# ka9q/ka9q-radio

Measured on NVIDIA H100. Metric: input Msamples/s through forward+filter+inverse at N channels, higher is better.
Workload: dtype f32

## Files before the change

include/ka9q_gpu.h:

```cpp
#ifndef KA9Q_GPU_H
#define KA9Q_GPU_H 1
#include <stddef.h>
#include <stdint.h>

#ifdef __cplusplus
extern "C" {
#endif

enum kgpu_type { KGPU_COMPLEX = 1, KGPU_REAL = 2 };
enum kgpu_format {
  KGPU_FMT_F32 = 0,
  KGPU_FMT_I16 = 1
};
enum kgpu_chan_flags {
  KGPU_CHAN_ISB = 1,
  KGPU_CHAN_BEAM = 4
};

typedef struct kgpu_master kgpu_master;
typedef struct kgpu_bank kgpu_bank;

struct kgpu_ingest_stats {
  unsigned long long energy;
  unsigned int clips;
  unsigned int pad;
};

const char *kgpu_last_error(void);
unsigned long long kgpu_launch_count(void);
int kgpu_profile_enable(int on);
int kgpu_profile_reset(void);
int kgpu_profile_kernels(void);
const char *kgpu_profile_name(int kernel);
int kgpu_profile_get(int kernel, double *total_ms, long *count);
int kgpu_device_count(void);
int kgpu_set_device(int device);

kgpu_master *kgpu_master_create(int L, int M, int in_type);
kgpu_master *kgpu_master_create_ex(int L, int M, int in_type);
kgpu_master *kgpu_master_create_any(int L, int M, int in_type);
int kgpu_master_plan(int L, int M, int in_type, char *buf, int buflen);
void kgpu_master_destroy(kgpu_master *m);
int kgpu_master_points(kgpu_master const *m);
int kgpu_master_bins(kgpu_master const *m);
long kgpu_master_spec_stride(kgpu_master const *m);
int kgpu_master_describe(kgpu_master const *m, char *buf, int buflen);

int kgpu_forward(kgpu_master *m, const void *d_in, int fmt, float scale, int derandomize, int nblocks,
                 void *d_spec, void *d_stats, void *stream);

int kgpu_unpack_airspy12(const void *d_packed, long sampcount, void *d_i16, void *d_stats, void *stream);

enum kgpu_raw8 {
  KGPU_RAW_U8 = 1,
  KGPU_RAW_S8 = 2
};
struct kgpu_block_stats {
  unsigned long long energy;
  unsigned int overs;
  unsigned int over_samples;
};
struct kgpu_scale_change {
  long long at;
  double scale;
};
int kgpu_unpack8(const void *d_raw, int fmt, int in_type, long history, long L, int nblocks, double scale,
                 const struct kgpu_scale_change *d_chg, int nchg, long long a0, void *d_out, void *d_stats, void *stream);
int kgpu_scale_i16(const void *d_in, int in_type, long count, long long a0, double scale, const struct kgpu_scale_change *d_chg,
                   int nchg, int derandomize, float *d_out, void *stream);
int kgpu_block_stats_i16(const void *d_in, int in_type, long history, long L, int nblocks, int derandomize, int limit,
                         void *d_stats, void *stream);

enum kgpu_iq_fmt {
  KGPU_IQ_S8 = 1,
  KGPU_IQ_S16 = 2
};
struct kgpu_iq_write {
  long long first;
  long long n;
  double scale;
  long long m[5];
  long long overs;
  long long last_over;
};
struct kgpu_iq_state {
  double dc_i, dc_q, sinphi, imbalance, gain_i, gain_q, secphi, tanphi;
};
struct kgpu_iq_params {
  int kind;
  double dc_alpha;
  double gp;
};
struct kgpu_iq_record {
  long long seq;
  long long n, sum_i, sum_q;
  double i_energy, q_energy, dotprod;
  long long overs;
  long long since_over;
  struct kgpu_iq_state state;
};
int kgpu_iq_moments(const void *d_raw, int fmt, long long a0, long count, struct kgpu_iq_write *d_tab, int cap,
                    long long w_lo, int nw, void *stream);
int kgpu_iq_scan(const struct kgpu_iq_write *d_tab, struct kgpu_iq_state *d_coef, int cap, long long w_from, int nw,
                 const struct kgpu_iq_params *params, struct kgpu_iq_record *d_rec, void *stream);
int kgpu_iq_apply(const void *d_raw, int fmt, long long a0, long count, const struct kgpu_iq_write *d_tab,
                  const struct kgpu_iq_state *d_coef, int cap, long long w_lo, int nw, void *d_out, void *stream);

int kgpu_master_set_notches(kgpu_master *m, int const *bins, double const *alpha, int n);
int kgpu_apply_notches(kgpu_master *m, void *d_spec, int nblocks, void *stream);

kgpu_bank *kgpu_bank_create(kgpu_master *m, int capacity);
void kgpu_bank_destroy(kgpu_bank *b);
int kgpu_bank_define(kgpu_bank *b, int idx, int olen);
int kgpu_bank_define_ex(kgpu_bank *b, int idx, int olen, int out_type);
int kgpu_bank_define_wide(kgpu_bank *b, int idx, int olen, int out_type);
int kgpu_bank_define_huge(kgpu_bank *b, int idx, int olen, int out_type);
int kgpu_bank_define_ext(kgpu_bank *b, int idx, int olen, int out_type);
int kgpu_bank_define_any(kgpu_bank *b, int idx, int olen, int out_type);
int kgpu_chan_plan(int points, int out_type, char *buf, int buflen);
int kgpu_bank_set_filter(kgpu_bank *b, int idx, double low, double high, double kaiser_beta);
int kgpu_bank_set_filter_on(kgpu_bank *b, int idx, double low, double high, double kaiser_beta, void *stream);
int kgpu_bank_set_response(kgpu_bank *b, int idx, float const *response);
int kgpu_bank_get_response(kgpu_bank *b, int idx, float *response);
int kgpu_bank_set_shift(kgpu_bank *b, int idx, int shift);
int kgpu_bank_set_flags(kgpu_bank *b, int idx, int flags);
int kgpu_bank_enable(kgpu_bank *b, int idx, int enabled);
int kgpu_bank_set_weights(kgpu_bank *b, int idx, double alpha_re, double alpha_im, double beta_re, double beta_im);
int kgpu_bank_set_osc(kgpu_bank *b, int idx, int enable, double phase_cycles, double freq_cps, double rate_cps2,
                      double block_adj_cycles);
int kgpu_bank_get_osc_phase(kgpu_bank *b, int idx, double *phase_cycles);
int kgpu_bank_set_block_counter(kgpu_bank *b, long counter);
long kgpu_bank_block_counter(kgpu_bank const *b);
int kgpu_bank_channels(kgpu_bank const *b);
long kgpu_bank_out_stride(kgpu_bank const *b);
long kgpu_bank_out_offset(kgpu_bank const *b, int idx);
int kgpu_bank_run(kgpu_bank *b, const void *d_spec, int nblocks, void *d_out, void *stream);
int kgpu_bank_run_ex(kgpu_bank *b, const void *d_spec, int nblocks, void *d_out, long out_pitch, float *d_power, void *stream);
int kgpu_bank_run_one(kgpu_bank *b, int idx, const void *d_spec, void *d_out, void *stream);
int kgpu_bank_run_one_ex(kgpu_bank *b, int idx, const void *d_spec, void *d_out, float *d_power , void *stream);
int kgpu_bank_noise(kgpu_bank *b, const void *d_spec, int nblocks, double samprate, double *d_n0, void *stream);

int kgpu_bank_fm_front(kgpu_bank *b, const void *d_out, long out_pitch, int nblocks, float *d_baseband, double *d_stats, void *stream);

int kgpu_bank_commit(kgpu_bank *b, void *stream);
int kgpu_use_static_kernels(int on);
int kgpu_use_cols_tma(int on);
int kgpu_cols_tma_fits(int L, int M, int in_type, int fmt, const void *d_in);

int kgpu_plan_radices(int len, int *radices, int max);
int kgpu_plan_split(long n, int *n1, int *n2);
int kgpu_plan_radices_ex(int len, int *radices, int max);
int kgpu_plan_split_ex(long n, int *n1, int *n2);

int kgpu_multicast_copy(const void *d_src, void *mc_dst, unsigned long long bytes, int nctas, void *stream);

typedef struct kgpu_spectrum kgpu_spectrum;
kgpu_spectrum *kgpu_spectrum_create(int fft_n, int in_type, int bin_count);
int kgpu_spectrum_set_window(kgpu_spectrum *s, float const *window);
int kgpu_spectrum_run(kgpu_spectrum *s, const void *d_ring, long ring_samples, long end, int fmt, float scale,
                      const struct kgpu_scale_change *d_chg, int nchg, long long end_index, int derandomize, int shift, int fft_avg, double overlap, float *d_bins, void *stream);
int kgpu_spectrum_run_narrow(kgpu_spectrum *s, const void *d_ring, long ring_size, long ring_idx, int fft_avg,
                             double overlap, float *d_bins, int *fft_avg_used, void *stream);
int kgpu_spectrum_ring_append(void *d_ring, long ring_size, long ring_idx, const void *d_src, long olen, void *stream);
int kgpu_spectrum_describe(kgpu_spectrum const *s, char *buf, int buflen);
void kgpu_spectrum_destroy(kgpu_spectrum *s);
int kgpu_spectrum_plan(int fft_n, int in_type, char *buf, int buflen);

double kgpu_algorithmic_bytes(kgpu_master const *m, kgpu_bank const *b, int fmt);

#ifdef __cplusplus
}
#endif
#endif
```

ka9q_radio_b200/capi.py:

```python
from __future__ import annotations

import ctypes as C
import os
import subprocess
from pathlib import Path

PKG = Path(__file__).resolve().parent
LIB_PATH = PKG / "libka9qgpu.so"

KGPU_COMPLEX, KGPU_REAL = 1, 2
KGPU_FMT_F32, KGPU_FMT_I16 = 0, 1
KGPU_RAW_U8, KGPU_RAW_S8 = 1, 2
KGPU_CHAN_ISB = 1
KGPU_CHAN_BEAM = 4

_lib = None


class KgpuError(RuntimeError):
    pass


def build(force: bool = False) -> None:
    if force or not LIB_PATH.exists():
        subprocess.run(["make", "-C", str(PKG / "csrc"), "-s"], check=True)


def load() -> C.CDLL:
    global _lib
    if _lib is not None:
        return _lib
    if not LIB_PATH.exists():
        raise KgpuError(
            f"{LIB_PATH} is missing: build it with `make -C ka9q_radio_b200/csrc` "
            "(python -c 'import __graft_entry__ as g; g.build()'). There is no CPU fallback."
        )
    L = C.CDLL(str(LIB_PATH))
    vp, i, d, f, l = C.c_void_p, C.c_int, C.c_double, C.c_float, C.c_long
    L.kgpu_last_error.restype = C.c_char_p
    L.kgpu_launch_count.restype = C.c_ulonglong
    L.kgpu_set_device.argtypes = [i]
    L.kgpu_master_create.restype = vp
    L.kgpu_master_create.argtypes = [i, i, i]
    L.kgpu_master_create_ex.restype = vp
    L.kgpu_master_create_ex.argtypes = [i, i, i]
    L.kgpu_master_create_any.restype = vp
    L.kgpu_master_create_any.argtypes = [i, i, i]
    L.kgpu_master_plan.argtypes = [i, i, i, C.c_char_p, i]
    L.kgpu_master_destroy.argtypes = [vp]
    L.kgpu_master_points.argtypes = [vp]
    L.kgpu_master_bins.argtypes = [vp]
    L.kgpu_master_spec_stride.argtypes = [vp]
    L.kgpu_master_spec_stride.restype = l
    L.kgpu_master_describe.argtypes = [vp, C.c_char_p, i]
    L.kgpu_forward.argtypes = [vp, vp, i, f, i, i, vp, vp, vp]
    L.kgpu_master_set_notches.argtypes = [vp, vp, vp, i]
    L.kgpu_apply_notches.argtypes = [vp, vp, i, vp]
    L.kgpu_bank_create.restype = vp
    L.kgpu_bank_create.argtypes = [vp, i]
    L.kgpu_bank_destroy.argtypes = [vp]
    L.kgpu_bank_define.argtypes = [vp, i, i]
    L.kgpu_bank_set_filter.argtypes = [vp, i, d, d, d]
    L.kgpu_bank_set_filter_on.argtypes = [vp, i, d, d, d, vp]
    L.kgpu_bank_set_response.argtypes = [vp, i, vp]
    L.kgpu_bank_get_response.argtypes = [vp, i, vp]
    L.kgpu_bank_set_shift.argtypes = [vp, i, i]
    L.kgpu_bank_set_flags.argtypes = [vp, i, i]
    L.kgpu_bank_enable.argtypes = [vp, i, i]
    L.kgpu_bank_channels.argtypes = [vp]
    L.kgpu_bank_out_stride.argtypes = [vp]
    L.kgpu_bank_out_stride.restype = l
    L.kgpu_bank_out_offset.argtypes = [vp, i]
    L.kgpu_bank_out_offset.restype = l
    L.kgpu_bank_run.argtypes = [vp, vp, i, vp, vp]
    L.kgpu_bank_run_one.argtypes = [vp, i, vp, vp, vp]
    L.kgpu_bank_commit.argtypes = [vp, vp]
    L.kgpu_unpack_airspy12.argtypes = [vp, l, vp, vp, vp]
    L.kgpu_unpack8.argtypes = [vp, i, i, l, l, i, d, vp, i, C.c_longlong, vp, vp, vp]
    L.kgpu_block_stats_i16.argtypes = [vp, i, l, l, i, i, i, vp, vp]
    ll = C.c_longlong
    L.kgpu_iq_moments.argtypes = [vp, i, ll, l, vp, i, ll, i, vp]
    L.kgpu_iq_scan.argtypes = [vp, vp, i, ll, i, vp, vp, vp]
    L.kgpu_iq_apply.argtypes = [vp, i, ll, l, vp, vp, i, ll, i, vp, vp]
    L.kgpu_bank_define_ex.argtypes = [vp, i, i, i]
    L.kgpu_bank_define_wide.argtypes = [vp, i, i, i]
    L.kgpu_bank_define_huge.argtypes = [vp, i, i, i]
    L.kgpu_bank_define_ext.argtypes = [vp, i, i, i]
    L.kgpu_bank_define_any.argtypes = [vp, i, i, i]
    L.kgpu_chan_plan.argtypes = [i, i, C.c_char_p, i]
    L.kgpu_bank_set_weights.argtypes = [vp, i, d, d, d, d]
    L.kgpu_bank_set_osc.argtypes = [vp, i, i, d, d, d, d]
    L.kgpu_bank_get_osc_phase.argtypes = [vp, i, vp]
    L.kgpu_bank_set_block_counter.argtypes = [vp, l]
    L.kgpu_bank_block_counter.argtypes = [vp]
    L.kgpu_bank_block_counter.restype = l
    L.kgpu_bank_run_ex.argtypes = [vp, vp, i, vp, l, vp, vp]
    L.kgpu_bank_run_one_ex.argtypes = [vp, i, vp, vp, vp, vp]
    L.kgpu_bank_noise.argtypes = [vp, vp, i, d, vp, vp]
    L.kgpu_bank_fm_front.argtypes = [vp, vp, l, i, vp, vp, vp]
    L.kgpu_use_static_kernels.argtypes = [i]
    L.kgpu_use_cols_tma.argtypes = [i]
    L.kgpu_cols_tma_fits.argtypes = [i, i, i, i, vp]
    L.kgpu_profile_enable.argtypes = [i]
    L.kgpu_profile_name.argtypes = [i]
    L.kgpu_profile_name.restype = C.c_char_p
    L.kgpu_profile_get.argtypes = [i, vp, vp]
    L.kgpu_plan_radices.argtypes = [i, vp, i]
    L.kgpu_plan_split.argtypes = [l, vp, vp]
    L.kgpu_plan_radices_ex.argtypes = [i, vp, i]
    L.kgpu_plan_split_ex.argtypes = [l, vp, vp]
    L.kgpu_multicast_copy.argtypes = [vp, vp, C.c_ulonglong, i, vp]
    L.kgpu_algorithmic_bytes.argtypes = [vp, vp, i]
    L.kgpu_algorithmic_bytes.restype = d
    L.kgpu_spectrum_create.restype = vp
    L.kgpu_spectrum_create.argtypes = [i, i, i]
    L.kgpu_spectrum_set_window.argtypes = [vp, vp]
    L.kgpu_spectrum_run.argtypes = [vp, vp, l, l, i, f, vp, i, C.c_longlong, i, i, i, d, vp, vp]
    L.kgpu_spectrum_run_narrow.argtypes = [vp, vp, l, l, i, d, vp, vp, vp]
    L.kgpu_spectrum_ring_append.argtypes = [vp, l, l, vp, l, vp]
    L.kgpu_spectrum_describe.argtypes = [vp, C.c_char_p, i]
    L.kgpu_spectrum_destroy.argtypes = [vp]
    L.kgpu_spectrum_plan.argtypes = [i, i, C.c_char_p, i]
    _lib = L
    return L


def exported_symbols() -> list[str]:
    import re

    hdr = (PKG.parent / "include" / "ka9q_gpu.h").read_text()
    hdr = re.sub(r"/\*.*?\*/", " ", hdr, flags=re.S)
    return sorted(set(re.findall(r"\b(kgpu_[a-z0-9_]+)\s*\(", hdr)))


def profile_snapshot() -> dict[str, tuple[float, int]]:
    L = load()
    out = {}
    for k in range(L.kgpu_profile_kernels()):
        ms, cnt = C.c_double(0), C.c_long(0)
        L.kgpu_profile_get(k, C.cast(C.pointer(ms), C.c_void_p), C.cast(C.pointer(cnt), C.c_void_p))
        out[L.kgpu_profile_name(k).decode()] = (ms.value, cnt.value)
    return out


def plan_radices(length: int, extended: bool = False) -> list[int]:
    out = (C.c_int * 16)()
    fn = load().kgpu_plan_radices_ex if extended else load().kgpu_plan_radices
    n = fn(length, C.cast(out, C.c_void_p), 16)
    if n < 0:
        raise KgpuError(f"length {length} cannot be planned")
    return [out[k] for k in range(n)]


def plan_split(n: int, extended: bool = False) -> tuple[int, int]:
    a, b = C.c_int(0), C.c_int(0)
    fn = load().kgpu_plan_split_ex if extended else load().kgpu_plan_split
    if fn(n, C.cast(C.pointer(a), C.c_void_p), C.cast(C.pointer(b), C.c_void_p)) != 0:
        raise KgpuError(f"{n} points cannot be split")
    return a.value, b.value


def check(rc: int, what: str = "") -> int:
    if rc < 0:
        raise KgpuError(f"{what}: {load().kgpu_last_error().decode()}")
    return rc


def unpack8(d_raw: int, fmt: int, in_type: int, history: int, L: int, nblocks: int, scale: float, d_out: int,
            d_stats: int = 0, stream: int = 0) -> None:
    check(load().kgpu_unpack8(d_raw, fmt, in_type, history, L, nblocks, scale, None, 0, 0, d_out, d_stats or None,
                              stream or None), "kgpu_unpack8")


def block_stats_i16(d_in: int, in_type: int, history: int, L: int, nblocks: int, d_stats: int, derandomize: bool = False,
                    limit: int = 32767, stream: int = 0) -> None:
    check(load().kgpu_block_stats_i16(d_in, in_type, history, L, nblocks, int(derandomize), limit, d_stats, stream or None),
          "kgpu_block_stats_i16")


KGPU_IQ_S8, KGPU_IQ_S16 = 1, 2
IQ_HACKRF, IQ_FUNCUBE = 1, 2


class IqParams(C.Structure):
    _fields_ = [("kind", C.c_int), ("dc_alpha", C.c_double), ("gp", C.c_double)]


def iq_moments(d_raw: int, fmt: int, a0: int, count: int, d_tab: int, cap: int, w_lo: int, nw: int, stream: int = 0) -> None:
    check(load().kgpu_iq_moments(d_raw, fmt, a0, count, d_tab, cap, w_lo, nw, stream or None), "kgpu_iq_moments")


def iq_scan(d_tab: int, d_coef: int, cap: int, w_from: int, nw: int, kind: int, dc_alpha: float, gp: float, d_rec: int,
            stream: int = 0) -> None:
    p = IqParams(kind, dc_alpha, gp)
    check(load().kgpu_iq_scan(d_tab, d_coef, cap, w_from, nw, C.byref(p), d_rec, stream or None), "kgpu_iq_scan")


def iq_apply(d_raw: int, fmt: int, a0: int, count: int, d_tab: int, d_coef: int, cap: int, w_lo: int, nw: int, d_out: int,
             stream: int = 0) -> None:
    check(load().kgpu_iq_apply(d_raw, fmt, a0, count, d_tab, d_coef, cap, w_lo, nw, d_out, stream or None), "kgpu_iq_apply")


MASTER_DIRECT, MASTER_EXTENDED, MASTER_BLUESTEIN = 0, 1, 2


def plan_master(L: int, M: int, in_type: int) -> tuple[int, str]:
    buf = C.create_string_buffer(512)
    return check(load().kgpu_master_plan(L, M, in_type, buf, 512), "kgpu_master_plan"), buf.value.decode()


CHAN_DIRECT, CHAN_WIDE, CHAN_HUGE, CHAN_EXTENDED, CHAN_BLUESTEIN = 0, 1, 2, 3, 4


def chan_plan(points: int, out_type: int = KGPU_COMPLEX) -> tuple[int, str]:
    buf = C.create_string_buffer(512)
    return check(load().kgpu_chan_plan(points, out_type, buf, 512), "kgpu_chan_plan"), buf.value.decode()


class Master:

    def __init__(self, L: int, M: int, in_type: int, extended: bool = False, any_length: bool = False):
        self.lib = load()
        if any_length:
            what = "kgpu_master_create_any"
        else:
            what = "kgpu_master_create_ex" if extended else "kgpu_master_create"
        self.h = getattr(self.lib, what)(L, M, in_type)
        if not self.h:
            raise KgpuError(f"{what}: " + self.lib.kgpu_last_error().decode())
        self.L, self.M, self.in_type = L, M, in_type
        self.N = self.lib.kgpu_master_points(self.h)
        self.bins = self.lib.kgpu_master_bins(self.h)
        self.spec_stride = self.lib.kgpu_master_spec_stride(self.h)

    def describe(self) -> str:
        buf = C.create_string_buffer(512)
        self.lib.kgpu_master_describe(self.h, buf, 512)
        return buf.value.decode()

    def forward(self, d_in: int, fmt: int, scale: float, nblocks: int, d_spec: int, stream: int = 0,
                derandomize: bool = False, d_stats: int = 0) -> None:
        check(self.lib.kgpu_forward(self.h, d_in, fmt, scale, int(derandomize), nblocks, d_spec, d_stats or None,
                                    stream or None), "kgpu_forward")

    def set_notches(self, bins, alpha=0.01) -> None:
        bins = list(bins) + [0]
        n = len(bins)
        b = (C.c_int * n)(*bins)
        a = (C.c_double * n)(*([alpha] * n))
        check(self.lib.kgpu_master_set_notches(self.h, C.cast(b, C.c_void_p), C.cast(a, C.c_void_p), n), "set_notches")

    def apply_notches(self, d_spec: int, nblocks: int, stream: int = 0) -> None:
        check(self.lib.kgpu_apply_notches(self.h, d_spec, nblocks, stream or None), "kgpu_apply_notches")

    def close(self):
        if self.h:
            self.lib.kgpu_master_destroy(self.h)
            self.h = None


class Bank:

    def __init__(self, master: Master, capacity: int):
        self.lib = load()
        self.m = master
        self.h = self.lib.kgpu_bank_create(master.h, capacity)
        if not self.h:
            raise KgpuError("kgpu_bank_create: " + self.lib.kgpu_last_error().decode())

    def define(self, idx, olen, out_type=KGPU_COMPLEX) -> int:
        return check(self.lib.kgpu_bank_define_ex(self.h, idx, olen, out_type), "kgpu_bank_define_ex")

    def define_wide(self, idx, olen, out_type=KGPU_COMPLEX) -> int:
        return check(self.lib.kgpu_bank_define_wide(self.h, idx, olen, out_type), "kgpu_bank_define_wide")

    def define_huge(self, idx, olen, out_type=KGPU_COMPLEX) -> int:
        return check(self.lib.kgpu_bank_define_huge(self.h, idx, olen, out_type), "kgpu_bank_define_huge")

    def define_ext(self, idx, olen, out_type=KGPU_COMPLEX) -> int:
        return check(self.lib.kgpu_bank_define_ext(self.h, idx, olen, out_type), "kgpu_bank_define_ext")

    def define_any(self, idx, olen, out_type=KGPU_COMPLEX) -> int:
        return check(self.lib.kgpu_bank_define_any(self.h, idx, olen, out_type), "kgpu_bank_define_any")

    def set_weights(self, idx, i_weight=1.0, q_weight=0.0):
        a = 0.5 * complex(i_weight) - 1j * complex(q_weight)
        b = 0.5 * complex(i_weight) + 1j * complex(q_weight)
        check(self.lib.kgpu_bank_set_weights(self.h, idx, a.real, a.imag, b.real, b.imag), "kgpu_bank_set_weights")

    def set_osc(self, idx, enable, phase=0.0, freq=0.0, rate=0.0, block_adj=0.0):
        check(self.lib.kgpu_bank_set_osc(self.h, idx, int(enable), phase, freq, rate, block_adj), "kgpu_bank_set_osc")

    def osc_phase(self, idx) -> float:
        v = C.c_double(0)
        check(self.lib.kgpu_bank_get_osc_phase(self.h, idx, C.cast(C.pointer(v), C.c_void_p)), "kgpu_bank_get_osc_phase")
        return v.value

    @property
    def block_counter(self) -> int:
        return self.lib.kgpu_bank_block_counter(self.h)

    @block_counter.setter
    def block_counter(self, v: int):
        check(self.lib.kgpu_bank_set_block_counter(self.h, int(v)), "kgpu_bank_set_block_counter")

    def fm_front(self, d_out: int, nblocks: int, d_baseband: int, d_stats: int, stream: int = 0):
        check(self.lib.kgpu_bank_fm_front(self.h, d_out, 0, nblocks, d_baseband, d_stats, stream or None), "kgpu_bank_fm_front")

    def noise(self, d_spec: int, nblocks: int, samprate: float, d_n0: int, stream: int = 0):
        check(self.lib.kgpu_bank_noise(self.h, d_spec, nblocks, samprate, d_n0, stream or None), "kgpu_bank_noise")

    def set_filter(self, idx, low, high, beta):
        check(self.lib.kgpu_bank_set_filter(self.h, idx, low, high, beta), "kgpu_bank_set_filter")

    def set_response(self, idx, resp):
        import numpy as np

        r = np.ascontiguousarray(resp, np.complex64)
        check(self.lib.kgpu_bank_set_response(self.h, idx, r.ctypes.data), "kgpu_bank_set_response")

    def get_response(self, idx, points):
        import numpy as np

        r = np.empty(points, np.complex64)
        check(self.lib.kgpu_bank_get_response(self.h, idx, r.ctypes.data), "kgpu_bank_get_response")
        return r

    def set_shift(self, idx, shift):
        check(self.lib.kgpu_bank_set_shift(self.h, idx, int(shift)), "kgpu_bank_set_shift")

    def set_flags(self, idx, flags):
        check(self.lib.kgpu_bank_set_flags(self.h, idx, int(flags)), "kgpu_bank_set_flags")

    def enable(self, idx, on=True):
        check(self.lib.kgpu_bank_enable(self.h, idx, int(on)), "kgpu_bank_enable")

    @property
    def out_stride(self) -> int:
        return self.lib.kgpu_bank_out_stride(self.h)

    def out_offset(self, idx) -> int:
        return self.lib.kgpu_bank_out_offset(self.h, idx)

    def run(self, d_spec: int, nblocks: int, d_out: int, stream: int = 0, d_power: int = 0):
        check(self.lib.kgpu_bank_run_ex(self.h, d_spec, nblocks, d_out, 0, d_power or None, stream or None), "kgpu_bank_run")

    def run_one(self, idx, d_spec: int, d_out: int, stream: int = 0):
        check(self.lib.kgpu_bank_run_one(self.h, idx, d_spec, d_out, stream or None), "kgpu_bank_run_one")

    def algorithmic_bytes(self, fmt) -> float:
        return self.lib.kgpu_algorithmic_bytes(self.m.h, self.h, fmt)

    def close(self):
        if self.h:
            self.lib.kgpu_bank_destroy(self.h)
            self.h = None


SPECTRUM_R2C, SPECTRUM_COMPLEX, SPECTRUM_BLUESTEIN = 0, 1, 2


def spectrum_plan(fft_n: int, in_type: int) -> tuple[int, str]:
    buf = C.create_string_buffer(256)
    return check(load().kgpu_spectrum_plan(fft_n, in_type, buf, 256), "kgpu_spectrum_plan"), buf.value.decode()


def spectrum_ring_append(ring, ring_idx: int, block, stream: int = 0) -> int:
    import torch

    if not (ring.is_cuda and ring.is_contiguous() and ring.dtype == torch.float32 and ring.shape[-1] == 2):
        raise ValueError("ring must be a contiguous float32 CUDA tensor of (re, im) pairs")
    size = ring.numel() // 2
    if isinstance(block, int):
        src, n = None, block
    else:
        if not (block.is_cuda and block.is_contiguous() and block.dtype == torch.float32 and block.shape[-1] == 2):
            raise ValueError("block must be a contiguous float32 CUDA tensor of (re, im) pairs")
        src, n = block.data_ptr(), block.numel() // 2
    check(load().kgpu_spectrum_ring_append(ring.data_ptr(), size, int(ring_idx), src, n, stream or None),
          "kgpu_spectrum_ring_append")
    return (int(ring_idx) + n) % size


class Spectrum:

    def __init__(self, fft_n: int, in_type: int, bin_count: int):
        self.lib = load()
        self.h = self.lib.kgpu_spectrum_create(fft_n, in_type, bin_count)
        if not self.h:
            raise KgpuError("kgpu_spectrum_create: " + self.lib.kgpu_last_error().decode())
        self.fft_n, self.in_type, self.bin_count = fft_n, in_type, bin_count

    def describe(self) -> str:
        buf = C.create_string_buffer(256)
        self.lib.kgpu_spectrum_describe(self.h, buf, 256)
        return buf.value.decode()

    def set_window(self, window) -> None:
        import numpy as np

        w = np.ascontiguousarray(window, np.float32)
        if w.shape != (self.fft_n,):
            raise ValueError(f"window needs {self.fft_n} floats")
        check(self.lib.kgpu_spectrum_set_window(self.h, w.ctypes.data), "kgpu_spectrum_set_window")

# ... 37 lines not shown
```

ka9q_radio_b200/csrc/fft_static.cuh:

```cuda
#pragma once
#include "fft_radix.cuh"

namespace kfft {

template <int LEN, int... RS> struct SPlan {
  static constexpr int len = LEN;
  static constexpr int nst = sizeof...(RS);
  static constexpr int rad_arr[sizeof...(RS) > 0 ? sizeof...(RS) : 1] = {RS...};
  static constexpr int rad(int i) { return rad_arr[i]; }
  static constexpr int nsub(int i) {
    int n = LEN;
    for (int k = 0; k < i; k++) n /= rad_arr[k];
    return n;
  }
  static constexpr int stride(int i) { return nsub(i) / rad_arr[i]; }
  static constexpr int tw_off(int i) {
    int o = 0;
    for (int k = 0; k < i; k++)
      if (stride(k) > 1) o += (rad_arr[k] - 1) * stride(k);
    return o;
  }
  static constexpr bool valid() {
    int p = 1;
    for (int k = 0; k < nst; k++) p *= rad_arr[k];
    return p == LEN;
  }
};

template <class P, int I = 0> struct SlotOf {
  static __device__ __forceinline__ int run(int rem) {
    constexpr int R = P::rad(I), S = P::stride(I);
    int const q = rem / R;
    return (rem - q * R) * S + SlotOf<P, I + 1>::run(q);
  }
};
template <class P> struct SlotOf<P, P::nst> {
  static __device__ __forceinline__ int run(int) { return 0; }
};
template <class P> __device__ __forceinline__ int static_slot(int k) { return SlotOf<P>::run(k); }

template <class P> constexpr int static_tw_count() { return P::tw_off(P::nst); }

__device__ __forceinline__ int ldg_stream_b32(int const *p) {
  int v;
  asm volatile("ld.global.nc.L1::no_allocate.b32 %0, [%1];" : "=r"(v) : "l"(p));
  return v;
}
__device__ __forceinline__ float2 ldg_stream_f2(float2 const *p) {
  float2 v;
  asm volatile("ld.global.nc.L1::no_allocate.v2.f32 {%0, %1}, [%2];" : "=f"(v.x), "=f"(v.y) : "l"(p));
  return v;
}

template <class P, int I> struct StageGeom {
  static constexpr int R = P::rad(I), NSUB = P::nsub(I), S = P::stride(I), NB = P::len / R;
  static __device__ __forceinline__ void split(int u, int &b, int &j) {
    if (S == 1) {
      b = u;
      j = 0;
    } else {
      b = u / S;
      j = u - b * S;
    }
  }
};

template <class P, bool INV, int I, bool TWS, int ILP>
__device__ __forceinline__ void static_stage(float2 *__restrict__ col, float2 const *__restrict__ tw, int lane) {
  using G = StageGeom<P, I>;
  constexpr int R = G::R, NSUB = G::NSUB, S = G::S, NB = G::NB, NL = 32;
  constexpr int ITERS = (NB + NL - 1) / NL;
  float2 const *twi = tw + P::tw_off(I);
#pragma unroll
  for (int it0 = 0; it0 < ITERS; it0 += ILP) {
    float2 x[ILP][R];
    float2 *p[ILP];
    int jj[ILP];
    bool ok[ILP];
#pragma unroll
    for (int q = 0; q < ILP; q++) {
      int const u = lane + NL * (it0 + q);
      ok[q] = (it0 + q < ITERS) && ((NB % NL == 0) || it0 + q + 1 < ITERS || u < NB);
      int b, j;
      G::split(ok[q] ? u : 0, b, j);
      jj[q] = j;
      p[q] = col + b * NSUB + j;
      if (ok[q]) {
#pragma unroll
        for (int m = 0; m < R; m++) x[q][m] = p[q][m * S];
      }
    }
#pragma unroll
    for (int q = 0; q < ILP; q++) {
      if (ok[q]) {
        Dft<R, INV>::run(x[q]);
        if (S > 1) {
#pragma unroll
          for (int t = 1; t < R; t++) {
            float2 const w = TWS ? twi[(t - 1) * S + jj[q]] : __ldg(twi + (t - 1) * S + jj[q]);
            x[q][t] = INV ? cmulc(x[q][t], w) : cmul(x[q][t], w);
          }
        }
      }
    }
#pragma unroll
    for (int q = 0; q < ILP; q++) {
      if (ok[q]) {
#pragma unroll
        for (int t = 0; t < R; t++) p[q][t * S] = x[q][t];
      }
    }
  }
}

template <class P, bool INV, bool TWS = false, int ILP = 1, int I = 0> struct StaticFft {
  static __device__ __forceinline__ void run(float2 *col, float2 const *tw, int lane) {
    static_stage<P, INV, I, TWS, (P::rad(I) <= 12 ? ILP : 1)>(col, tw, lane);
    __syncwarp();
    StaticFft<P, INV, TWS, ILP, I + 1>::run(col, tw, lane);
  }
};
template <class P, bool INV, bool TWS, int ILP> struct StaticFft<P, INV, TWS, ILP, P::nst> {
  static __device__ __forceinline__ void run(float2 *, float2 const *, int) {}
};

__device__ __forceinline__ uint32_t smem_u32(void const *p) { return (uint32_t)__cvta_generic_to_shared(p); }
__device__ __forceinline__ void mbar_init(uint64_t *bar, int count) {
  asm volatile("mbarrier.init.shared::cta.b64 [%0], %1;" ::"r"(smem_u32(bar)), "r"(count));
}
__device__ __forceinline__ void mbar_fence_init() { asm volatile("fence.mbarrier_init.release.cluster;" ::: "memory"); }
__device__ __forceinline__ void mbar_expect_tx(uint64_t *bar, uint32_t bytes) {
  asm volatile("mbarrier.arrive.expect_tx.shared::cta.b64 _, [%0], %1;" ::"r"(smem_u32(bar)), "r"(bytes) : "memory");
}
__device__ __forceinline__ void bulk_g2s(void *dst, void const *src, uint32_t bytes, uint64_t *bar) {
  asm volatile("cp.async.bulk.shared::cluster.global.mbarrier::complete_tx::bytes [%0], [%1], %2, [%3];" ::"r"(smem_u32(dst)),
               "l"(src), "r"(bytes), "r"(smem_u32(bar))
               : "memory");
}
__device__ __forceinline__ void tensor_g2s_3d(void *dst, void const *map, int x, int y, int z, uint64_t *bar) {
  asm volatile("cp.async.bulk.tensor.3d.shared::cluster.global.tile.mbarrier::complete_tx::bytes [%0], [%1, {%2, %3, %4}], [%5];"
               ::"r"(smem_u32(dst)), "l"(map), "r"(x), "r"(y), "r"(z), "r"(smem_u32(bar))
               : "memory");
}
__device__ __forceinline__ void mbar_wait(uint64_t *bar, uint32_t parity) {
  asm volatile(
      "{\n\t.reg .pred p;\n\t"
      "WAIT_%=:\n\t"
      "mbarrier.try_wait.parity.shared::cta.b64 p, [%0], %1;\n\t"
      "@p bra DONE_%=;\n\t"
      "bra WAIT_%=;\n\t"
      "DONE_%=:\n\t}" ::"r"(smem_u32(bar)),
      "r"(parity)
      : "memory");
}

}
```

ka9q_radio_b200/csrc/fwd_cols_r36.cuh:

```cuda
#pragma once
#include <cuda.h>

#include "static_kernels_v2.cuh"

namespace kfft {

struct ColsR36Tables {
  float2 const *tw0;
  float2 const *twA;
  float2 const *twB;
};

__device__ __forceinline__ float2 r36_power(float2 const (&wb)[6], float2 const (&wa)[6], int t) {
  int const a = t / 6, b = t - 6 * a;
  if (a == 0) return wb[b];
  if (b == 0) return wa[a];
  return cmul(wa[a], wb[b]);
}

struct ColsR36Shape {
  static constexpr int BLK = 38, CP = 1378, T = 288;
  static constexpr size_t smem = sizeof(float2) * (size_t)(8 * CP + 360 + 80);
};

struct ColsR36Tma {
  static constexpr int BOX_ROWS = 216;
  static constexpr int F32_BOX_BYTES = BOX_ROWS * 64;
  static constexpr int I16_BOX_WORDS = 12, I16_BOX_BYTES = BOX_ROWS * I16_BOX_WORDS * 4;
  static constexpr int I16_ODD_OFF = 3 * I16_BOX_BYTES;
  static constexpr uint32_t bytes(int fmt) { return fmt == 0 ? 6 * F32_BOX_BYTES : 6 * I16_BOX_BYTES; }
};
static_assert(ColsR36Tma::bytes(0) + 112 <= sizeof(float2) * 8 * ColsR36Shape::CP &&
              ColsR36Tma::bytes(1) + 112 <= sizeof(float2) * 8 * ColsR36Shape::CP, "the raw tile lies in the float tile");
static_assert(ColsR36Tma::F32_BOX_BYTES % 128 == 0 && ColsR36Tma::I16_BOX_BYTES % 128 == 0, "box destinations 128-B aligned");

template <int FMT>
__device__ __forceinline__ float2 r36_ingest(int raw, int row, int col, int n2, Pass1Args const &a, unsigned long long &energy,
                                             unsigned int &clips) {
  int lo, hi;
  unpack_i16(raw, lo, hi);
  if (FMT == 2) {
    if (a.derandomize) {
      lo ^= (lo & 1) ? 0xfffffffe : 0;
      hi ^= (hi & 1) ? 0xfffffffe : 0;
    }
    if (a.stats && (long)row * n2 + col >= a.first_new) {
      energy += (unsigned long long)(lo * lo) + (unsigned long long)(hi * hi);
      clips += (lo > 32766 || lo < -32766) + (hi > 32766 || hi < -32766);
    }
  }
  return make_float2(i32_to_f32(lo), i32_to_f32(hi));
}

__device__ __forceinline__ void r36_stage0_store(float2 (&x)[36], float2 const *s_tw0, float2 *d, int ul) {
  constexpr int R = 36, BLK = ColsR36Shape::BLK;
  float2 wb[6], wa[6];
#pragma unroll
  for (int b = 1; b < 6; b++) {
    wb[b] = s_tw0[(b - 1) * 36 + ul];
    wa[b] = s_tw0[(4 + b) * 36 + ul];
  }
  d[0] = x[0];
#pragma unroll
  for (int t = 1; t < R; t++) d[t * BLK] = cmul(x[t], r36_power(wb, wa, t));
}

template <int FMT, int N2C, bool TMA>
__device__ __forceinline__ void fwd_cols_r36_body(Pass1Args const &a, ColsR36Tables const &tb, CUtensorMap const *tmap) {
  constexpr int R = 36, BLK = ColsR36Shape::BLK, CP = ColsR36Shape::CP;
  extern __shared__ __align__(16) unsigned char smem_raw[];
  float2 *tile = reinterpret_cast<float2 *>(smem_raw);
  float2 *s_tw0 = tile + 8 * CP;
  float2 *s_twB = s_tw0 + 360;
  __shared__ __align__(8) uint64_t tbar;
  int const tid = threadIdx.x;
  int const c = tid & 7, ul = tid >> 3;
  int const c0 = blockIdx.x * 8, blk = blockIdx.y;
  int const n2 = N2C ? N2C : a.n2;
  int const ld = N2C ? (N2C + 15) / 16 * 16 : a.mid_ld;
  int const ncols = min(8, n2 - c0);
  bool const col_ok = c < ncols;
  int const n2g = c0 + c;
  float2 *mycol = tile + c * CP;
  unsigned char *const rtile = smem_raw + ((0u - smem_u32(smem_raw)) & 127u);
  if (tid == 0) {
    mbar_init(&tbar, 1);
    mbar_fence_init();
    if constexpr (TMA) {
      using T = ColsR36Tma;
      mbar_expect_tx(&tbar, 360 * 8 + 80 * 8 + T::bytes(FMT));
      if (FMT == 0) {
#pragma unroll
        for (int k = 0; k < 6; k++) tensor_g2s_3d(rtile + k * T::F32_BOX_BYTES, tmap, 2 * c0, k * T::BOX_ROWS, blk, &tbar);
      } else {
#pragma unroll
        for (int k = 0; k < 3; k++) {
          tensor_g2s_3d(rtile + k * T::I16_BOX_BYTES, tmap, c0, k * T::BOX_ROWS, blk, &tbar);
          tensor_g2s_3d(rtile + T::I16_ODD_OFF + k * T::I16_BOX_BYTES, tmap, n2 + c0 - (n2 & 2), k * T::BOX_ROWS, blk, &tbar);
        }
      }
    } else {
      mbar_expect_tx(&tbar, 360 * 8 + 80 * 8);
    }
    bulk_g2s(s_tw0, tb.tw0, 360 * 8, &tbar);
    bulk_g2s(s_twB, tb.twB + (long)c0 * 10, 80 * 8, &tbar);
  }
  __syncthreads();
  float2 const twA = col_ok ? ldg_stream_f2(tb.twA + (long)n2g * 36 + ul) : make_float2(1.f, 0.f);

  unsigned long long energy = 0;
  unsigned int clips = 0;
  if constexpr (TMA) {
    float2 x[R];
    mbar_wait(&tbar, 0);
    if (col_ok) {
      if (FMT == 0) {
        float2 const *src = reinterpret_cast<float2 const *>(rtile) + ul * 8 + c;
#pragma unroll
        for (int m = 0; m < R; m++) x[m] = src[R * 8 * m];
      } else {
        using T = ColsR36Tma;
        int const odd = ul & 1;
        int const *src = reinterpret_cast<int const *>(rtile + odd * T::I16_ODD_OFF) + (ul >> 1) * T::I16_BOX_WORDS + c +
                         odd * (n2 & 2);
#pragma unroll
        for (int m = 0; m < R; m++)
          x[m] = r36_ingest<FMT>(src[(R / 2) * T::I16_BOX_WORDS * m], ul + R * m, n2g, n2, a, energy, clips);
      }
      Dft<R, false>::run(x);
    }
    __syncthreads();
    if (col_ok) r36_stage0_store(x, s_tw0, mycol + ul, ul);
  } else if (col_ok) {
    float2 x[R];
    if (FMT == 0) {
      float2 const *src = reinterpret_cast<float2 const *>(a.in) + (long)blk * a.hop + n2g + (long)ul * n2;
#pragma unroll
      for (int m = 0; m < R; m++) x[m] = ldg_stream_f2(src + (long)(R * m) * n2);
    } else {
      int const *src = reinterpret_cast<int const *>(a.in) + (long)blk * a.hop + n2g + (long)ul * n2;
      int raw[R];
#pragma unroll
      for (int m = 0; m < R; m++) raw[m] = ldg_stream_b32(src + (long)(R * m) * n2);
#pragma unroll
      for (int m = 0; m < R; m++) x[m] = r36_ingest<FMT>(raw[m], ul + R * m, n2g, n2, a, energy, clips);
    }
    mbar_wait(&tbar, 0);
    Dft<R, false>::run(x);
    r36_stage0_store(x, s_tw0, mycol + ul, ul);
  } else {
    mbar_wait(&tbar, 0);
  }
  if (FMT == 2 && a.stats) {
#pragma unroll
    for (int o = 16; o > 0; o >>= 1) {
      energy += __shfl_xor_sync(0xffffffffu, energy, o);
      clips += __shfl_xor_sync(0xffffffffu, clips, o);
    }
    if ((tid & 31) == 0 && (energy | clips)) {
      atomicAdd(&a.stats[blk].energy, energy);
      atomicAdd(&a.stats[blk].clips, clips);
    }
  }
  __syncthreads();

  if (col_ok) {
    float2 x[R];
    float4 const *p4 = reinterpret_cast<float4 const *>(mycol + ul * BLK);
#pragma unroll
    for (int m = 0; m < R / 2; m++) {
      float4 const v = p4[m];
      x[2 * m] = make_float2(v.x, v.y);
      x[2 * m + 1] = make_float2(v.z, v.w);
    }
    Dft<R, false>::run(x);
    float2 wb[6], wa[6];
#pragma unroll
    for (int b = 1; b < 6; b++) {
      wb[b] = s_twB[c * 10 + (b - 1)];
      wa[b] = s_twB[c * 10 + (4 + b)];
    }
    float2 const w0 = make_float2(twA.x * a.out_scale, twA.y * a.out_scale);
    float2 *dst = a.mid + (long)blk * 1296 * ld + n2g + (long)ul * ld;
    dst[0] = cmul(x[0], w0);
#pragma unroll
    for (int k = 1; k < R; k++) dst[(long)(R * k) * ld] = cmul(x[k], cmul(w0, r36_power(wb, wa, k)));
  }
}

template <int FMT, int N2C>
__global__ void __launch_bounds__(ColsR36Shape::T, 2) fwd_cols_r36(Pass1Args const a, ColsR36Tables const tb) {
  fwd_cols_r36_body<FMT, N2C, false>(a, tb, nullptr);
}
template <int FMT, int N2C>
__global__ void __launch_bounds__(ColsR36Shape::T, 2)
    fwd_cols_r36_tma(Pass1Args const a, ColsR36Tables const tb, const __grid_constant__ CUtensorMap tmap) {
  fwd_cols_r36_body<FMT, N2C, true>(a, tb, &tmap);
}

}
```

ka9q_radio_b200/csrc/fwd_kernels.cuh:

```cuda
#pragma once
#include "fft_tile.cuh"

namespace kfft {

constexpr int kTile = 8;
constexpr int kFwdThreads = kTile * 32;

struct IngestStats {
  unsigned long long energy;
  unsigned int clips;
  unsigned int pad;
};

struct Pass1Args {
  void const *in;
  long hop;
  int n1, n2;
  long nc;
  int plan;
  int pitch;
  float scale;
  int derandomize;
  long first_new;
  float2 *mid;
  IngestStats *stats;
  float out_scale;
  int mid_ld;
};

__device__ __forceinline__ float2 unit_root_f(long e, long n) {
  double s, c;
  sincospi(2.0 * (double)e / (double)n, &s, &c);
  return make_float2((float)c, (float)-s);
}

template <int FMT , bool EXT>
__device__ __forceinline__ void fwd_cols_body(Pass1Args const &a, TilePlan const &pl) {
  extern __shared__ __align__(16) unsigned char smem_raw[];
  float2 *tile = reinterpret_cast<float2 *>(smem_raw);
  int const rows_per_it = kFwdThreads / kTile;
  int const nit = (a.n1 + rows_per_it - 1) / rows_per_it;
  float2 *twA = tile + kTile * a.pitch;

  int const tid = threadIdx.x, lane = tid & 31, warp = tid >> 5;
  int const c = tid % kTile, r = tid / kTile;
  int const c0 = blockIdx.x * kTile;
  int const blk = blockIdx.y;
  int const ncols = min(kTile, a.n2 - c0);
  bool const col_ok = c < ncols;
  long const n2g = c0 + c;

  unsigned long long energy = 0;
  unsigned int clips = 0;
  constexpr int U = 8;
  if (FMT == 1) {
    int const *src = reinterpret_cast<int const *>(a.in) + (long)blk * a.hop + n2g;
    auto put = [&](int n1, int w) {
      short lo = (short)(w & 0xffff), hi = (short)((unsigned)w >> 16);
      if (a.derandomize) {
        lo ^= (short)((lo & 1) ? 0xfffe : 0);
        hi ^= (short)((hi & 1) ? 0xfffe : 0);
      }
      if (a.stats && (long)n1 * a.n2 + n2g >= a.first_new) {
        energy += (unsigned long long)((int)lo * lo) + (unsigned long long)((int)hi * hi);
        clips += (lo > 32766 || lo < -32766) + (hi > 32766 || hi < -32766);
      }
      tile[c * a.pitch + n1] = make_float2((float)lo * a.scale, (float)hi * a.scale);
    };
    int n1 = r;
    if (col_ok) {
      for (; n1 + (U - 1) * rows_per_it < a.n1; n1 += U * rows_per_it) {
        int w[U];
#pragma unroll
        for (int u = 0; u < U; u++) w[u] = __ldg(src + (long)(n1 + u * rows_per_it) * a.n2);
#pragma unroll
        for (int u = 0; u < U; u++) put(n1 + u * rows_per_it, w[u]);
      }
      for (; n1 < a.n1; n1 += rows_per_it) put(n1, __ldg(src + (long)n1 * a.n2));
    } else {
      for (; n1 < a.n1; n1 += rows_per_it) tile[c * a.pitch + n1] = make_float2(0.f, 0.f);
    }
  } else {
    float2 const *src = reinterpret_cast<float2 const *>(a.in) + (long)blk * a.hop + n2g;
    int n1 = r;
    if (col_ok) {
      for (; n1 + (U - 1) * rows_per_it < a.n1; n1 += U * rows_per_it) {
        float2 w[U];
#pragma unroll
        for (int u = 0; u < U; u++) w[u] = __ldg(src + (long)(n1 + u * rows_per_it) * a.n2);
#pragma unroll
        for (int u = 0; u < U; u++) tile[c * a.pitch + n1 + u * rows_per_it] = w[u];
      }
      for (; n1 < a.n1; n1 += rows_per_it) tile[c * a.pitch + n1] = __ldg(src + (long)n1 * a.n2);
    } else {
      for (; n1 < a.n1; n1 += rows_per_it) tile[c * a.pitch + n1] = make_float2(0.f, 0.f);
    }
  }
  float2 twB = make_float2(1.f, 0.f);
  if (col_ok) twB = unit_root_f((n2g * r) % a.nc, a.nc);
  for (int i = tid; i < kTile * nit; i += kFwdThreads) {
    int const cc = i / nit, it = i - cc * nit;
    long const e = ((long)(c0 + cc) * rows_per_it * it) % a.nc;
    twA[i] = unit_root_f(e, a.nc);
  }
  if (FMT == 1 && a.stats) {
#pragma unroll
    for (int o = 16; o > 0; o >>= 1) {
      energy += __shfl_xor_sync(0xffffffffu, energy, o);
      clips += __shfl_xor_sync(0xffffffffu, clips, o);
    }
    if (lane == 0 && (energy | clips)) {
      atomicAdd(&a.stats[blk].energy, energy);
      atomicAdd(&a.stats[blk].clips, clips);
    }
  }
  __syncthreads();

  if (warp < ncols) tile_fft<false, EXT>(pl, tile + warp * a.pitch, lane, 32, [] { __syncwarp(); });
  __syncthreads();

  if (col_ok) {
    float2 *dst = a.mid + (long)blk * a.nc + n2g;
    float2 const *colp = tile + c * a.pitch;
    float2 const *twc = twA + c * nit;
    constexpr int V = 4;
    int it = 0, k1 = r;
    for (; k1 + (V - 1) * rows_per_it < a.n1; k1 += V * rows_per_it, it += V) {
      int slot[V];
      float2 v[V];
#pragma unroll
      for (int u = 0; u < V; u++) slot[u] = __ldg(pl.perm + k1 + u * rows_per_it);
#pragma unroll
      for (int u = 0; u < V; u++) v[u] = cmul(colp[slot[u]], cmul(twB, twc[it + u]));
#pragma unroll
      for (int u = 0; u < V; u++) dst[(long)(k1 + u * rows_per_it) * a.n2] = v[u];
    }
    for (; k1 < a.n1; k1 += rows_per_it, it++)
      dst[(long)k1 * a.n2] = cmul(colp[__ldg(pl.perm + k1)], cmul(twB, twc[it]));
  }
}

template <int FMT>
__global__ void __launch_bounds__(kFwdThreads, 2) fwd_cols_kernel(Pass1Args const a) {
  fwd_cols_body<FMT, false>(a, c_plans[a.plan]);
}
template <int FMT>
__global__ void __launch_bounds__(kFwdThreads, 2) fwd_cols_ext(Pass1Args const a, __grid_constant__ TilePlan const pl) {
  fwd_cols_body<FMT, true>(a, pl);
}

enum RowKind : int { kRowEmpty = 0, kRowPair = 1, kRowSelf0 = 2, kRowSelfMid = 3, kRowPlain = 4 };
struct RowItem {
  int kind;
  int row_a;
  int row_b;
};

__device__ __forceinline__ RowItem row_item(int p, int n1, bool real_split) {
  RowItem it;
  if (!real_split) {
    it.kind = p < n1 ? kRowPlain : kRowEmpty;
    it.row_a = p;
    it.row_b = 0;
    return it;
  }
  it.row_a = p;
  it.row_b = n1 - p;
  if (p == 0) it.kind = kRowSelf0, it.row_b = 0;
  else if (2 * p < n1) it.kind = kRowPair;
  else if (2 * p == n1) it.kind = kRowSelfMid, it.row_b = p;
  else it.kind = kRowEmpty, it.row_a = it.row_b = 0;
  return it;
}

struct Pass2Args {
  float2 const *mid;
  int n1, n2;
  long nc;
  int plan;
  int pitch;
  int real_split;
  float2 const *rootD;
  float2 *spec;
  long spec_stride;
  int mid_ld;
};

__global__ void __launch_bounds__(kFwdThreads, 2) fwd_rows_kernel(Pass2Args const a) {
  TilePlan const &pl = c_plans[a.plan];
#define KFFT_ROWS_EXT false
#include "fwd_rows_body.cuh"
#undef KFFT_ROWS_EXT
}
__global__ void __launch_bounds__(kFwdThreads, 2) fwd_rows_ext(Pass2Args const a, __grid_constant__ TilePlan const pl) {
#define KFFT_ROWS_EXT true
#include "fwd_rows_body.cuh"
#undef KFFT_ROWS_EXT
}

struct NotchDev {
  int bin;
  int pad;
  double re, im;
  double alpha;
};
__global__ void notch_kernel(NotchDev *list, int n, int sequential, float2 *spec, long spec_stride, int nblocks) {
  int const i = blockIdx.x * blockDim.x + threadIdx.x;
  if (sequential) {
    if (i != 0) return;
    for (int b = 0; b < nblocks; b++)
      for (int e = 0; e < n; e++) {
        float2 *p = spec + (long)b * spec_stride + list[e].bin;
        float2 v = *p;
        list[e].re += list[e].alpha * ((double)v.x - list[e].re);
        list[e].im += list[e].alpha * ((double)v.y - list[e].im);
        *p = make_float2((float)((double)v.x - list[e].re), (float)((double)v.y - list[e].im));
      }
    return;
  }
  if (i >= n) return;
  NotchDev nd = list[i];
  for (int b = 0; b < nblocks; b++) {
    float2 *p = spec + (long)b * spec_stride + nd.bin;
    float2 v = *p;
    nd.re += nd.alpha * ((double)v.x - nd.re);
    nd.im += nd.alpha * ((double)v.y - nd.im);
    *p = make_float2((float)((double)v.x - nd.re), (float)((double)v.y - nd.im));
  }
  list[i].re = nd.re;
  list[i].im = nd.im;
}

}
```

ka9q_radio_b200/csrc/kgpu.cu:

```cuda
#include <cuda_runtime.h>
#include <cudaTypedefs.h>
#include <math.h>
#include <stdarg.h>
#include <stdio.h>
#include <stdlib.h>
#include <string.h>
#include <algorithm>
#include <complex>
#include <atomic>
#include <map>
#include <mutex>
#include <string>
#include <vector>

#include "../../include/ka9q_gpu.h"
#include "chan_kernels.cuh"
#include "chan_huge.cuh"
#include "chan_wide.cuh"
#include "fwd_kernels.cuh"
#include "noise_kernel.cuh"
#include "plan.cuh"
#include "static_kernels.cuh"
#include "static_kernels_v2.cuh"
#include "fwd_cols_r36.cuh"
#include "fwd_2s.cuh"
#include "spectrum_kernels.cuh"
#include "bluestein_master.cuh"
#include "bluestein_chan.cuh"
#include "raw_ingest.cuh"
#include "iq_correct.cuh"

using namespace kfft;

static thread_local std::string g_err;
static std::atomic<unsigned long long> g_launches{0};

static std::atomic<int> g_static_on{1};
extern "C" int kgpu_use_static_kernels(int on) {
  g_static_on.store(on != 0);
  return 0;
}
static std::atomic<int> g_cols_tma{-1};
extern "C" int kgpu_use_cols_tma(int on) {
  g_cols_tma.store(on != 0);
  return 0;
}
static bool cols_tma_on() {
  int v = g_cols_tma.load();
  if (v < 0) {
    char const *e = getenv("KA9Q_COLS_TMA");
    g_cols_tma.compare_exchange_strong(v, (e && *e) ? (atoi(e) != 0) : 1);
    v = g_cols_tma.load();
  }
  return v != 0;
}

static int fail(char const *fmt, ...) {
  char buf[512];
  va_list ap;
  va_start(ap, fmt);
  vsnprintf(buf, sizeof buf, fmt, ap);
  va_end(ap);
  g_err = buf;
  return -1;
}
#define CUDA_OK(expr)                                                                    \
  do {                                                                                   \
    cudaError_t e_ = (expr);                                                             \
    if (e_ != cudaSuccess) return fail("%s: %s (%s:%d)", #expr, cudaGetErrorString(e_), __FILE__, __LINE__); \
  } while (0)
#define CUDA_OKP(expr)                                                                   \
  do {                                                                                   \
    cudaError_t e_ = (expr);                                                             \
    if (e_ != cudaSuccess) {                                                             \
      fail("%s: %s (%s:%d)", #expr, cudaGetErrorString(e_), __FILE__, __LINE__);         \
      return nullptr;                                                                    \
    }                                                                                    \
  } while (0)

static int allow_smem(const void *func, size_t bytes) {
  if (bytes <= 48 * 1024) return 0;
  static std::mutex mu;
  static std::map<std::pair<int, const void *>, size_t> granted;
  int dev = 0;
  CUDA_OK(cudaGetDevice(&dev));
  std::lock_guard<std::mutex> lk(mu);
  size_t &g = granted[{dev, func}];
  if (bytes <= g) return 0;
  CUDA_OK(cudaFuncSetAttribute(func, cudaFuncAttributeMaxDynamicSharedMemorySize, (int)bytes));
  g = bytes;
  return 0;
}

struct StreamBuf {
  void *p = nullptr;
  size_t bytes = 0;
};
static int grow(StreamBuf &s, size_t bytes, cudaStream_t st, char const *who) {
  if (s.bytes >= bytes) return 0;
  if (cudaStreamSynchronize(st) != cudaSuccess)
    return fail("%s: cudaStreamSynchronize: %s", who, cudaGetErrorString(cudaGetLastError()));
  cudaFree(s.p);
  s.p = nullptr;
  s.bytes = 0;
  cudaError_t const e = cudaMalloc(&s.p, bytes);
  if (e != cudaSuccess) {
    s.p = nullptr;
    return fail("%s: cudaMalloc(%zu): %s", who, bytes, cudaGetErrorString(e));
  }
  s.bytes = bytes;
  return 0;
}

enum KernelId { K_FWD_COLS = 0, K_FWD_ROWS, K_CHAN, K_NOTCH, K_RESPONSE, K_NOISE, K_COUNT };
static char const *const kKernelNames[K_COUNT] = {"fwd_cols", "fwd_rows", "chan", "notch", "response_fft", "noise"};
struct ProfRec {
  cudaEvent_t a, b;
  int kid;
};
static std::atomic<int> g_prof_on{0};
static std::mutex g_prof_mu;
static std::vector<ProfRec> g_prof_pending;
static std::vector<cudaEvent_t> g_prof_pool;
static double g_prof_ms[K_COUNT];
static long g_prof_cnt[K_COUNT];

static cudaEvent_t prof_event() {
  if (!g_prof_pool.empty()) {
    cudaEvent_t e = g_prof_pool.back();
    g_prof_pool.pop_back();
    return e;
  }
  cudaEvent_t e;
  cudaEventCreate(&e);
  return e;
}
struct ProfScope {
  ProfRec r;
  cudaStream_t st;
  bool on;
  ProfScope(int kid, cudaStream_t s) : st(s), on(g_prof_on.load() != 0) {
    if (!on) return;
    std::lock_guard<std::mutex> lk(g_prof_mu);
    r.a = prof_event();
    r.b = prof_event();
    r.kid = kid;
    cudaEventRecord(r.a, st);
  }
  ~ProfScope() {
    if (!on) return;
    cudaEventRecord(r.b, st);
    std::lock_guard<std::mutex> lk(g_prof_mu);
    g_prof_pending.push_back(r);
  }
};
static void prof_drain() {
  std::lock_guard<std::mutex> lk(g_prof_mu);
  for (ProfRec &r : g_prof_pending) {
    float ms = 0;
    if (cudaEventSynchronize(r.b) == cudaSuccess && cudaEventElapsedTime(&ms, r.a, r.b) == cudaSuccess) {
      g_prof_ms[r.kid] += ms;
      g_prof_cnt[r.kid]++;
    }
    g_prof_pool.push_back(r.a);
    g_prof_pool.push_back(r.b);
  }
  g_prof_pending.clear();
}
extern "C" int kgpu_profile_enable(int on) {
  g_prof_on.store(on != 0);
  return 0;
}
extern "C" int kgpu_profile_reset(void) {
  prof_drain();
  for (int i = 0; i < K_COUNT; i++) {
    g_prof_ms[i] = 0;
    g_prof_cnt[i] = 0;
  }
  return 0;
}
extern "C" int kgpu_profile_kernels(void) { return K_COUNT; }
extern "C" const char *kgpu_profile_name(int kid) { return (kid >= 0 && kid < K_COUNT) ? kKernelNames[kid] : ""; }
extern "C" int kgpu_profile_get(int kid, double *total_ms, long *count) {
  if (kid < 0 || kid >= K_COUNT) return -1;
  prof_drain();
  if (total_ms) *total_ms = g_prof_ms[kid];
  if (count) *count = g_prof_cnt[kid];
  return 0;
}

extern "C" const char *kgpu_last_error(void) { return g_err.c_str(); }
extern "C" unsigned long long kgpu_launch_count(void) { return g_launches.load(); }
__global__ void __launch_bounds__(256) mc_push_kernel(float4 const *__restrict__ src, float4 *mc_dst, size_t n16) {
  size_t const stride = (size_t)gridDim.x * 256;
  size_t i = (size_t)blockIdx.x * 256 + threadIdx.x;
  for (; i + 3 * stride < n16; i += 4 * stride) {
    float4 v[4];
#pragma unroll
    for (int q = 0; q < 4; q++)
      asm volatile("ld.global.nc.L1::no_allocate.v4.f32 {%0,%1,%2,%3}, [%4];"
                   : "=f"(v[q].x), "=f"(v[q].y), "=f"(v[q].z), "=f"(v[q].w)
                   : "l"(src + i + q * stride));
#pragma unroll
    for (int q = 0; q < 4; q++)
      asm volatile("multimem.st.relaxed.sys.global.v4.f32 [%0], {%1,%2,%3,%4};" ::"l"(mc_dst + i + q * stride), "f"(v[q].x),
                   "f"(v[q].y), "f"(v[q].z), "f"(v[q].w)
                   : "memory");
  }
  for (; i < n16; i += stride) {
    float4 v;
    asm volatile("ld.global.nc.L1::no_allocate.v4.f32 {%0,%1,%2,%3}, [%4];" : "=f"(v.x), "=f"(v.y), "=f"(v.z), "=f"(v.w) : "l"(src + i));
    asm volatile("multimem.st.relaxed.sys.global.v4.f32 [%0], {%1,%2,%3,%4};" ::"l"(mc_dst + i), "f"(v.x), "f"(v.y), "f"(v.z), "f"(v.w)
                 : "memory");
  }
  __threadfence_system();
}
extern "C" int kgpu_multicast_copy(const void *d_src, void *mc_dst, unsigned long long bytes, int nctas, void *stream) {
  if (!d_src || !mc_dst || (bytes & 15) || ((uintptr_t)d_src & 15) || ((uintptr_t)mc_dst & 15))
    return fail("kgpu_multicast_copy: pointers and size must be multiples of 16 bytes");
  if (bytes == 0) return 0;
  if (nctas <= 0) nctas = 64;
  mc_push_kernel<<<nctas, 256, 0, (cudaStream_t)stream>>>((float4 const *)d_src, (float4 *)mc_dst, (size_t)(bytes / 16));
  g_launches++;
  CUDA_OK(cudaGetLastError());
  return 0;
}

__global__ void __launch_bounds__(256) airspy_unpack_kernel(uint32_t const *__restrict__ up, long ngroups, uint4 *__restrict__ out,
                                                            IngestStats *stats) {
  long const g = (long)blockIdx.x * 256 + threadIdx.x;
  unsigned long long energy = 0;
  unsigned int clips = 0;
  if (g < ngroups) {
    uint32_t const w0 = __ldg(up + 3 * g), w1 = __ldg(up + 3 * g + 1), w2 = __ldg(up + 3 * g + 2);
    uint32_t s[8] = {w0 >> 20, w0 >> 8, (w0 << 4) | (w1 >> 28), w1 >> 16, w1 >> 4, (w1 << 8) | (w2 >> 24), w2 >> 12, w2};
    int x[8];
#pragma unroll
    for (int j = 0; j < 8; j++) {
      x[j] = (int)(s[j] & 0xfffu) - 2048;
      clips += (x[j] == 2047 || x[j] <= -2047);
      energy += (unsigned long long)(x[j] * x[j]);
    }
    uint4 o;
    o.x = (uint32_t)(x[0] & 0xffff) | ((uint32_t)x[1] << 16);
    o.y = (uint32_t)(x[2] & 0xffff) | ((uint32_t)x[3] << 16);
    o.z = (uint32_t)(x[4] & 0xffff) | ((uint32_t)x[5] << 16);
    o.w = (uint32_t)(x[6] & 0xffff) | ((uint32_t)x[7] << 16);
    out[g] = o;
  }
  if (stats) {
#pragma unroll
    for (int o = 16; o > 0; o >>= 1) {
      energy += __shfl_xor_sync(0xffffffffu, energy, o);
      clips += __shfl_xor_sync(0xffffffffu, clips, o);
    }
    if ((threadIdx.x & 31) == 0 && (energy | clips)) {
      atomicAdd(&stats->energy, energy);
      atomicAdd(&stats->clips, clips);
    }
  }
}
extern "C" int kgpu_unpack_airspy12(const void *d_packed, long sampcount, void *d_i16, void *d_stats, void *stream) {
  if (!d_packed || !d_i16 || sampcount < 0 || (sampcount & 7)) return fail("kgpu_unpack_airspy12: sample count must be a multiple of 8");
  if (((uintptr_t)d_i16 & 15) || ((uintptr_t)d_packed & 3)) return fail("kgpu_unpack_airspy12: output must be 16-byte aligned");
  if (sampcount == 0) return 0;
  cudaStream_t st = (cudaStream_t)stream;
  if (d_stats) CUDA_OK(cudaMemsetAsync(d_stats, 0, sizeof(IngestStats), st));
  long const ng = sampcount / 8;
  airspy_unpack_kernel<<<(unsigned)((ng + 255) / 256), 256, 0, st>>>((uint32_t const *)d_packed, ng, (uint4 *)d_i16, (IngestStats *)d_stats);
  g_launches++;
  CUDA_OK(cudaGetLastError());
  return 0;
}

static_assert(sizeof(ScaleChange) == sizeof(kgpu_scale_change), "raw_ingest.cuh mirrors include/ka9q_gpu.h");
extern "C" int kgpu_unpack8(const void *d_raw, int fmt, int in_type, long history, long L, int nblocks, double scale,
                            const kgpu_scale_change *d_chg, int nchg, long long a0, void *d_out, void *d_stats, void *stream) {
  if (!d_raw || !d_out || history < 0 || nblocks < 0 || (nblocks > 0 && L < 1) || nblocks >= 65535 || nchg < 0 || (nchg && !d_chg) ||
      (fmt != KGPU_RAW_U8 && fmt != KGPU_RAW_S8) || (in_type != KGPU_REAL && in_type != KGPU_COMPLEX))
    return fail("kgpu_unpack8: bad arguments");
  cudaStream_t st = (cudaStream_t)stream;
  BlockStats *stats = (BlockStats *)d_stats;
  if (stats && nblocks) CUDA_OK(cudaMemsetAsync(stats, 0, sizeof(BlockStats) * (size_t)nblocks, st));
  long const longest = std::max(nblocks ? L : 0L, history);
  if (longest == 0) return 0;
  dim3 const g((unsigned)((longest + kRawThreads - 1) / kRawThreads), (unsigned)nblocks + 1);
  bool const s8 = fmt == KGPU_RAW_S8, cplx = in_type == KGPU_COMPLEX;
  auto const k = s8 ? (cplx ? unpack8_kernel<true, true> : unpack8_kernel<true, false>)
                    : (cplx ? unpack8_kernel<false, true> : unpack8_kernel<false, false>);
  k<<<g, kRawThreads, 0, st>>>((uint8_t const *)d_raw, history, L, nblocks, scale, (ScaleChange const *)d_chg, nchg, a0,
                               (float *)d_out, stats);
  g_launches++;
  CUDA_OK(cudaGetLastError());
  return 0;
}

extern "C" int kgpu_scale_i16(const void *d_in, int in_type, long count, long long a0, double scale, const kgpu_scale_change *d_chg,
                              int nchg, int derandomize, float *d_out, void *stream) {
  if (!d_in || !d_out || count < 0 || nchg < 0 || (nchg && !d_chg) || (in_type != KGPU_REAL && in_type != KGPU_COMPLEX))
    return fail("kgpu_scale_i16: bad arguments");
  if (count == 0) return 0;
  auto const k = in_type == KGPU_COMPLEX ? scale_i16_kernel<true> : scale_i16_kernel<false>;
  k<<<(unsigned)((count + kRawThreads - 1) / kRawThreads), kRawThreads, 0, (cudaStream_t)stream>>>(
      (short const *)d_in, count, a0, scale, (ScaleChange const *)d_chg, nchg, derandomize != 0, d_out);
  g_launches++;
  CUDA_OK(cudaGetLastError());
  return 0;
}

extern "C" int kgpu_block_stats_i16(const void *d_in, int in_type, long history, long L, int nblocks, int derandomize, int limit,
                                    void *d_stats, void *stream) {
  if (!d_in || !d_stats || history < 0 || L < 1 || nblocks < 1 || nblocks >= 65535 || limit < 1 ||
      (in_type != KGPU_REAL && in_type != KGPU_COMPLEX))
    return fail("kgpu_block_stats_i16: bad arguments");
  cudaStream_t st = (cudaStream_t)stream;
  CUDA_OK(cudaMemsetAsync(d_stats, 0, sizeof(BlockStats) * (size_t)nblocks, st));
  dim3 const g((unsigned)((L + kRawThreads - 1) / kRawThreads), (unsigned)nblocks);
  auto const k = in_type == KGPU_COMPLEX ? block_stats_i16_kernel<true> : block_stats_i16_kernel<false>;
  k<<<g, kRawThreads, 0, st>>>((short const *)d_in, history, L, derandomize != 0, limit, (BlockStats *)d_stats);
  g_launches++;
  CUDA_OK(cudaGetLastError());
  return 0;
}

static_assert(sizeof(IqWrite) == sizeof(kgpu_iq_write) && sizeof(IqState) == sizeof(kgpu_iq_state) &&
                  sizeof(IqRecord) == sizeof(kgpu_iq_record),
              "iq_correct.cuh mirrors include/ka9q_gpu.h");
static bool iq_args(const void *d_raw, int fmt, long count, const void *d_tab, int cap, int nw) {
  return d_raw && d_tab && count >= 0 && cap > 0 && nw > 0 && nw <= cap && (fmt == KGPU_IQ_S8 || fmt == KGPU_IQ_S16) &&
         (count + kIqChunk - 1) / kIqChunk < 0x7fffffffL;
}

extern "C" int kgpu_iq_moments(const void *d_raw, int fmt, long long a0, long count, kgpu_iq_write *d_tab, int cap,
                               long long w_lo, int nw, void *stream) {
  if (!iq_args(d_raw, fmt, count, d_tab, cap, nw) || a0 < 0 || w_lo < 0) return fail("kgpu_iq_moments: bad arguments");
  if (count == 0) return 0;
  auto const k = fmt == KGPU_IQ_S16 ? iq_moments_kernel<true> : iq_moments_kernel<false>;
  k<<<(unsigned)((count + kIqChunk - 1) / kIqChunk), kIqThreads, 0, (cudaStream_t)stream>>>(d_raw, a0, count, (IqWrite *)d_tab,
                                                                                           cap, w_lo, nw);
  g_launches++;
  CUDA_OK(cudaGetLastError());
  return 0;
}

extern "C" int kgpu_iq_scan(const kgpu_iq_write *d_tab, kgpu_iq_state *d_coef, int cap, long long w_from, int nw,
                            const kgpu_iq_params *params, kgpu_iq_record *d_rec, void *stream) {
  if (!d_tab || !d_coef || !d_rec || !params || cap < 2 || nw < 0 || nw >= cap || w_from < 0 ||
      (params->kind != 1 && params->kind != 2))
    return fail("kgpu_iq_scan: bad arguments");
  if (nw == 0) return 0;
  IqParams const p = {params->kind, params->dc_alpha, params->gp};
  iq_scan_kernel<<<1, 1, 0, (cudaStream_t)stream>>>((IqWrite const *)d_tab, (IqState *)d_coef, cap, w_from, nw, p,
                                                    (IqRecord *)d_rec);
  g_launches++;
  CUDA_OK(cudaGetLastError());
  return 0;
}

extern "C" int kgpu_iq_apply(const void *d_raw, int fmt, long long a0, long count, const kgpu_iq_write *d_tab,
                             const kgpu_iq_state *d_coef, int cap, long long w_lo, int nw, void *d_out, void *stream) {
  if (!iq_args(d_raw, fmt, count, d_tab, cap, nw) || !d_coef || !d_out || w_lo < 0) return fail("kgpu_iq_apply: bad arguments");
  if (count == 0) return 0;
  auto const k = fmt == KGPU_IQ_S16 ? iq_apply_kernel<true> : iq_apply_kernel<false>;
  k<<<(unsigned)((count + kIqChunk - 1) / kIqChunk), kIqThreads, 0, (cudaStream_t)stream>>>(
      d_raw, a0, count, (IqWrite const *)d_tab, (IqState const *)d_coef, cap, w_lo, nw, (float2 *)d_out);
  g_launches++;
  CUDA_OK(cudaGetLastError());
  return 0;
}

extern "C" int kgpu_device_count(void) {
  int n = 0;
  if (cudaGetDeviceCount(&n) != cudaSuccess) return 0;
  return n;
}
extern "C" int kgpu_set_device(int device) {
  CUDA_OK(cudaSetDevice(device));
  return 0;
}

namespace kfft {

static int const kRadixSet[] = {25, 24, 20, 16, 15, 12, 10, 9, 8, 7, 6, 5, 4, 3, 2};
static int const kRadixSetExt[] = {25, 24, 20, 16, 15, 12, 10, 9, 8, 7, 6, 5, 4, 3, 2, 23, 19, 17, 13, 11};

static_assert(kMaxChanPoints >= kMaxTileLen, "every tile length must also be a valid channel length");
constexpr int plannable_lengths(int max) {
  int count = 0;
  for (int n = 1; n <= max; n++) {
    int v = n;
    for (int p : {2, 3, 5, 7})
      while (v % p == 0) v /= p;
    count += (v == 1);
  }
  return count;
}
static_assert(plannable_lengths(kMaxChanPoints) <= kMaxPlans, "the plan registry must hold every plannable length");

static void search(int const *set, int nset, int n, int start, std::vector<int> &cur, std::vector<int> &best,
                   int &best_sum) {
  if (n == 1) {
    int sum = 0;
    for (int r : cur) sum += r;
    if (best.empty() || cur.size() < best.size() || (cur.size() == best.size() && sum < best_sum)) {
      best = cur;
      best_sum = sum;
    }
    return;
  }
  if ((int)cur.size() >= kMaxStages) return;
  if (!best.empty() && cur.size() + 1 > best.size()) return;
  for (int i = start; i < nset; i++) {
    int const r = set[i];
    if (n % r) continue;
    cur.push_back(r);
    search(set, nset, n / r, i, cur, best, best_sum);
    cur.pop_back();
  }
// ... 30 lines not shown
  p.nstages = (int)rad.size();
  std::vector<float2> tw;
  int n = len;
  for (int i = 0; i < p.nstages; i++) {
    int const r = rad[i], s = n / r;
    p.radix[i] = r;
    p.sub[i] = n;
    p.stride[i] = s;
    p.magic[i] = (s > 1) ? (uint32_t)(((1ull << 32) + (unsigned)s - 1) / (unsigned)s) : 0u;
    p.tw_off[i] = (int)tw.size();
    if (s > 1)
      for (int t = 1; t < r; t++)
        for (int j = 0; j < s; j++) {
          long double const ang = -2.0L * M_PIl * (long double)((long)j * t % n) / (long double)n;
          tw.push_back(make_float2((float)cosl(ang), (float)sinl(ang)));
        }
    n = s;
  }
  std::vector<uint16_t> perm((size_t)len);
  for (int k = 0; k < len; k++) {
    int rem = k, slot = 0;
    for (int i = 0; i < p.nstages; i++) {
      int const t = rem % p.radix[i];
      rem /= p.radix[i];
      slot += t * p.stride[i];
    }
    perm[k] = (uint16_t)slot;
  }
  float2 *d_tw = nullptr;
  uint16_t *d_perm = nullptr;
  tw.push_back(make_float2(0.f, 0.f));
  tw.push_back(make_float2(0.f, 0.f));
  p.tw = nullptr;
  p.perm = nullptr;
  auto upload = [&]() -> int {
    CUDA_OK(cudaMalloc(&d_tw, sizeof(float2) * tw.size()));
    CUDA_OK(cudaMalloc(&d_perm, sizeof(uint16_t) * (size_t)len));
    CUDA_OK(cudaMemcpy(d_tw, tw.data(), sizeof(float2) * tw.size(), cudaMemcpyHostToDevice));
    CUDA_OK(cudaMemcpy(d_perm, perm.data(), sizeof(uint16_t) * (size_t)len, cudaMemcpyHostToDevice));
    return 0;
  };
  if (upload()) {
    cudaFree(d_tw);
    cudaFree(d_perm);
    return -1;
  }
  p.tw = d_tw;
  p.perm = d_perm;
  return 0;
}
static void free_tile_plan(TilePlan &p) {
  cudaFree((void *)p.tw);
  cudaFree((void *)p.perm);
  p.tw = nullptr;
  p.perm = nullptr;
}

int get_tile_plan(int len) {
  std::lock_guard<std::mutex> lk(g_plan_mu);
  for (size_t i = 0; i < g_plans.size(); i++)
    if (g_plans[i].len == len) return (int)i;
  std::vector<int> rad;
  if (len > 1) rad = choose_radices(len);
  if (len < 1 || len > kMaxChanPoints || (len > 1 && rad.empty()))
    return fail("%d-point transform cannot be planned (factors 2, 3, 5, 7; at most %d points)", len, kMaxChanPoints);
  if ((int)g_plans.size() >= kMaxPlans) return fail("plan registry full (%d plans)", kMaxPlans);
  TilePlan p;
  if (make_tile_plan(len, rad, p)) return -1;
  int const idx = (int)g_plans.size();
  cudaError_t const e = cudaMemcpyToSymbol(c_plans, &p, sizeof p, sizeof(TilePlan) * (size_t)idx);
  if (e != cudaSuccess) {
    free_tile_plan(p);
    return fail("cudaMemcpyToSymbol(c_plans): %s", cudaGetErrorString(e));
  }
  PlanSlot sl;
  sl.len = len;
  sl.host = p;
  g_plans.push_back(sl);
  return idx;
}
TilePlan const *host_tile_plan(int idx) { return &g_plans[(size_t)idx].host; }

static bool plannable(int len) { return len == 1 || (len <= kMaxTileLen && !choose_radices(len).empty()); }
static bool plannable_ext(int len) { return len == 1 || (len <= kMaxTileLen && !choose_radices_ext(len).empty()); }

template <bool (*Plannable)(int)> static bool split_with(long n, Split2 *out) {
  long best = -1;
  for (long d = (long)floor(sqrt((double)n) + 1e-9); d >= 1; d--) {
    if (n % d) continue;
    long const a = n / d;
    if (a > kMaxTileLen) break;
    if (Plannable((int)a) && Plannable((int)d)) {
      best = d;
      break;
    }
  }
  if (best < 0) return false;
  out->n1 = (int)(n / best);
  out->n2 = (int)best;
  return true;
}
bool choose_split(long n, Split2 *out) { return split_with<plannable>(n, out); }
bool choose_split_ext(long n, Split2 *out) { return split_with<plannable_ext>(n, out); }

constexpr bool smooth7(long n) {
  for (long p : {2, 3, 5, 7})
    while (n % p == 0) n /= p;
  return n == 1;
}
constexpr bool wide_fits(long n) {
  long d = 1;
  while ((d + 1) * (d + 1) <= n) d++;
  for (; d >= 1; d--) {
    if (n % d) continue;
    if (n / d > kMaxTileLen) return false;
    if (smooth7(n / d) && smooth7(d)) return wide_smem_bytes((int)(n / d), (int)d) <= kChanSmemLimit;
  }
  return false;
}
constexpr bool all_wide_fit(long lo, long hi) {
  for (long n = lo; n <= hi; n++)
    if (smooth7(n) && !wide_fits(n)) return false;
  return true;
}
constexpr long next_smooth7(long n) {
  while (!smooth7(n)) n++;
  return n;
}
static_assert(all_wide_fit(kMaxChanPoints + 1, kMaxWideChanPoints), "a wide length up to the maximum does not fit");
static_assert(!wide_fits(next_smooth7(kMaxWideChanPoints + 1)), "kMaxWideChanPoints is below what shared memory holds");

static int plan_slot(TilePlan const &p, int k) {
  int slot = 0;
  for (int i = 0; i < p.nstages; i++) {
    slot += (k % p.radix[i]) * p.stride[i];
    k /= p.radix[i];
  }
  return slot;
}

static int wide_twiddles(WideGeom &g, TilePlan const &p2) {
  long const points = (long)g.n1 * g.n2;
  std::vector<float2> tw((size_t)points);
  for (int j2 = 0; j2 < g.n2; j2++) {
    int const c = plan_slot(p2, j2);
    for (int k1 = 0; k1 < g.n1; k1++) {
      long double const ang = -2.0L * M_PIl * (long double)((long)k1 * j2) / (long double)points;
      tw[(size_t)k1 * g.n2 + c] = make_float2((float)cosl(ang), (float)sinl(ang));
    }
  }
  float2 *d_tw = nullptr;
  if (cudaMalloc(&d_tw, sizeof(float2) * tw.size()) != cudaSuccess ||
      cudaMemcpy(d_tw, tw.data(), sizeof(float2) * tw.size(), cudaMemcpyHostToDevice) != cudaSuccess) {
    cudaFree(d_tw);
    return fail("%ld-point transform: twiddle upload failed", points);
  }
  g.tw = d_tw;
  return 0;
}

constexpr bool huge_fits(long n) {
  long d = 1;
  while ((d + 1) * (d + 1) <= n) d++;
  for (; d >= 1; d--) {
    if (n % d) continue;
    if (n / d > kMaxTileLen) return false;
    if (smooth7(n / d) && smooth7(d)) return huge_smem_bytes((int)(n / d)) <= kChanSmemLimit && huge_smem_bytes((int)d) <= kChanSmemLimit;
  }
  return false;
}
constexpr long huge_lengths(long lo, long hi) {
  long count = 0;
  for (long a = 1; a <= hi; a *= 2)
    for (long b = a; b <= hi; b *= 3)
      for (long c = b; c <= hi; c *= 5)
        for (long e = c; e <= hi; e *= 7)
          if (e > lo) {
            if (!huge_fits(e)) return -1;
            count++;
          }
  return count;
}
static_assert(huge_lengths(kMaxWideChanPoints, kMaxHugeChanPoints) == 806, "a huge length does not split or fit");

constexpr bool smooth23(long n) {
  for (long p : {2, 3, 5, 7, 11, 13, 17, 19, 23})
    while (n % p == 0) n /= p;
  return n == 1;
}
constexpr bool extended(long n) { return smooth23(n) && !smooth7(n); }
constexpr bool wide_fits_ext(long n) {
  long d = 1;
  while ((d + 1) * (d + 1) <= n) d++;
  for (; d >= 1; d--) {
    if (n % d) continue;
    if (n / d > kMaxTileLen) return false;
    if (smooth23(n / d) && smooth23(d)) return wide_smem_bytes((int)(n / d), (int)d) <= kChanSmemLimit;
  }
  return false;
}
constexpr long ext_lengths(long lo, long hi, bool wide) {
  long count = 0;
  for (long n = lo; n <= hi; n++)
    if (extended(n)) {
      if (wide && !wide_fits_ext(n)) return -1;
      count++;
    }
  return count;
}
static_assert(ext_lengths(2, kMaxChanPoints, false) == 863, "extended channel lengths up to kMaxChanPoints");
static_assert(ext_lengths(kMaxChanPoints + 1, kMaxWideChanPoints, true) == 1032, "an extended wide length does not split or fit");

static long factor_above7(long n) {
  long big = 1;
  for (long p = 2; p * p <= n; p++)
    while (n % p == 0) {
      n /= p;
      if (p > 7) big = p;
    }
  return n > 7 ? std::max(big, n) : big;
}

static bool forward_split(long nc, bool ext, Split2 *sp) {
  if (!(ext ? choose_split_ext(nc, sp) : choose_split(nc, sp))) return false;
  size_t const smem1 = sizeof(float2) * ((size_t)kTile * column_pitch(sp->n1) + (size_t)kTile * ((sp->n1 + 31) / 32));
  size_t const smem2 = sizeof(float2) * ((size_t)kTile * column_pitch(sp->n2));
  return smem1 <= (size_t)kChanSmemLimit && smem2 <= (size_t)kChanSmemLimit;
}

struct Bluestein {
  long n = 0;
  long P = 0;
  Split2 sp{};
  float2 *d_b = nullptr;
};
static bool bluestein_shape(long n, Bluestein *b) {
  long const limit = (long)kMaxTileLen * kMaxTileLen;
  for (long p = 2 * n - 1; p <= limit; p++)
    if (smooth7(p) && forward_split(p, false, &b->sp)) {
      b->n = n;
      b->P = p;
      return true;
    }
  return false;
}

static void host_dft(std::complex<double> *x, long n, std::complex<double> const *tw, long d) {
  if (n == 1) return;
  int const r = n % 2 == 0 ? 2 : n % 3 == 0 ? 3 : n % 5 == 0 ? 5 : 7;
  long const m = n / r;
  std::vector<std::complex<double>> t((size_t)n);
  for (long j = 0; j < m; j++)
    for (int q = 0; q < r; q++) t[(size_t)(q * m + j)] = x[j * r + q];
  for (int q = 0; q < r; q++) host_dft(t.data() + q * m, m, tw, d * r);
  for (long k = 0; k < m; k++)
    for (int s = 0; s < r; s++) {
      long const kk = k + s * m;
      std::complex<double> acc = t[(size_t)k];
      for (int q = 1; q < r; q++) acc += t[(size_t)(q * m + k)] * tw[(size_t)(((long)q * kk) % n * d)];
      x[kk] = acc;
    }
}

static std::vector<float2> bluestein_bspec(long n, long P) {
  std::vector<std::complex<double>> bd((size_t)P), tw((size_t)P);
  for (long m = 0; m < n; m++) {
    long double const ang = M_PIl * (long double)((m * m) % (2 * n)) / (long double)n;
    std::complex<double> const v((double)cosl(ang), (double)sinl(ang));
    bd[(size_t)m] = v;
    if (m) bd[(size_t)(P - m)] = v;
  }
  for (long e2 = 0; e2 < P; e2++) {
    long double const ang = -2.0L * M_PIl * (long double)e2 / (long double)P;
    tw[(size_t)e2] = std::complex<double>((double)cosl(ang), (double)sinl(ang));
  }
  host_dft(bd.data(), P, tw.data(), 1);
  std::vector<float2> b((size_t)P);
  for (long k = 0; k < P; k++) b[(size_t)k] = make_float2((float)bd[(size_t)k].real(), (float)bd[(size_t)k].imag());
  return b;
}
}

enum ColsKernel { COLS_GENERIC, COLS_R36, COLS_2S };
enum RowsKernel { ROWS_GENERIC, ROWS_V2, ROWS_2S };

struct kgpu_master {
  int L, M, N, in_type, bins;
  long nc;
  Split2 sp;
  int plan1, plan2, pitch1, pitch2;
  long spec_stride;
  int n_item_ctas = 0;
  int n_rows_ctas = 0;
  ColsKernel cols = COLS_GENERIC;
  RowsKernel rows = ROWS_GENERIC;
  bool halved = false;
  int n1c = 0, n2c = 0;
  int mid_ld = 0;
  float2 *d_rootD = nullptr;
  float2 *d_rootC = nullptr;
  float2 *d_tw0 = nullptr, *d_twA = nullptr, *d_twB = nullptr;
  float2 *d_rtw0 = nullptr;
  StreamBuf mid;
  size_t smem1 = 0, smem2 = 0;
  bool ext = false;
  TilePlan xplan1{}, xplan2{};
  kgpu_master *bs = nullptr;
  Bluestein blue;
  StreamBuf b_in, b_out;
  int b_chunk = 0;
  NotchDev *d_notch = nullptr;
  int n_notch = 0;
  int notch_sequential = 0;
};

using ColsR36Fn = void (*)(Pass1Args, ColsR36Tables);
using ColsR36TmaFn = void (*)(Pass1Args, ColsR36Tables, CUtensorMap);
using Cols2sFn = void (*)(Pass1Args, Cols2sTables);
using RowsV2Fn = void (*)(Pass2Args, FwdTables);
using Cols2s = Cols2sShape<25, 32>;
using Rows2s = Rows2sShape<25, 25>;
static ColsR36Fn cols_r36_kernel(kgpu_master const *m, int f) {
  static ColsR36Fn const k[2][3] = {{fwd_cols_r36<0, 0>, fwd_cols_r36<1, 0>, fwd_cols_r36<2, 0>},
                                    {fwd_cols_r36<0, 1250>, fwd_cols_r36<1, 1250>, fwd_cols_r36<2, 1250>}};
  return k[m->n2c == 1250][f];
}
static ColsR36TmaFn cols_r36_tma_kernel(kgpu_master const *m, int f) {
  static ColsR36TmaFn const k[2][3] = {{fwd_cols_r36_tma<0, 0>, fwd_cols_r36_tma<1, 0>, fwd_cols_r36_tma<2, 0>},
                                       {fwd_cols_r36_tma<0, 1250>, fwd_cols_r36_tma<1, 1250>, fwd_cols_r36_tma<2, 1250>}};
  return k[m->n2c == 1250][f];
}
static Cols2sFn cols_2s_kernel(int f) {
  static Cols2sFn const k[3] = {fwd_cols_2s<0, 25, 32>, fwd_cols_2s<1, 25, 32>, fwd_cols_2s<2, 25, 32>};
  return k[f];
}
static RowsV2Fn rows_v2_kernel(kgpu_master const *m) {
  if (m->in_type == KGPU_REAL) return m->halved ? fwd_rows_v2<true, 1296, true> : fwd_rows_v2<true, 0, false>;
  return m->n1c ? fwd_rows_v2<false, 1296, false> : fwd_rows_v2<false, 0, false>;
}
static int rows_v2_threads(kgpu_master const *m) { return m->in_type == KGPU_REAL ? RowsV2Shape<true>::T : RowsV2Shape<false>::T; }
static size_t rows_v2_smem(kgpu_master const *m) {
  return m->in_type == KGPU_REAL ? RowsV2Shape<true>::smem : RowsV2Shape<false>::smem;
}

static int upload(float2 **d, std::vector<float2> const &v) {
  CUDA_OK(cudaMalloc(d, sizeof(float2) * v.size()));
  CUDA_OK(cudaMemcpy(*d, v.data(), sizeof(float2) * v.size(), cudaMemcpyHostToDevice));
  return 0;
}

static int bluestein_upload(Bluestein *b) {
  if (upload(&b->d_b, bluestein_bspec(b->n, b->P)) == 0) return 0;
  cudaFree(b->d_b);
  b->d_b = nullptr;
  return -1;
}

static void master_geometry(kgpu_master *m, int L, int M, int in_type) {
  m->L = L;
  m->M = M;
  m->N = L + M - 1;
  m->in_type = in_type;
  m->bins = (in_type == KGPU_COMPLEX) ? m->N : m->N / 2 + 1;
  m->nc = (in_type == KGPU_COMPLEX) ? m->N : m->N / 2;
  m->spec_stride = ((long)m->bins + 3) / 4 * 4;
}

static void master_shape(kgpu_master *m, int L, int M, int in_type, Split2 const &sp, bool ext) {
  master_geometry(m, L, M, in_type);
  m->sp = sp;
  m->ext = ext;
  m->pitch1 = column_pitch(sp.n1);
  m->pitch2 = column_pitch(sp.n2);
  int const nit = (sp.n1 + 31) / 32;
  m->smem1 = sizeof(float2) * ((size_t)kTile * m->pitch1 + (size_t)kTile * nit);
  m->smem2 = sizeof(float2) * ((size_t)kTile * m->pitch2);
  int const n1 = sp.n1, n2 = sp.n2;
  bool const real = in_type == KGPU_REAL;
  if (ext) {
    m->mid_ld = n2;
    m->n_item_ctas = m->n_rows_ctas = real ? (n1 / 2 + 1 + 3) / 4 : (n1 + 7) / 8;
    return;
  }
  if (!real && n1 == 800 && n2 == 625) {
    m->cols = COLS_2S;
    m->rows = ROWS_2S;
  } else {
    if (n1 == 1296) m->cols = COLS_R36, m->n2c = (n2 == 1250) ? 1250 : 0;
    if (n2 == 1250) m->rows = ROWS_V2, m->n1c = (n1 == 1296) ? 1296 : 0;
  }
  m->halved = real && m->cols == COLS_R36 && m->rows == ROWS_V2;
  bool const padded = m->cols == COLS_2S || (m->cols == COLS_R36 && m->rows == ROWS_V2);
  m->mid_ld = padded ? (n2 + 15) / 16 * 16 : n2;
  m->n_item_ctas = real ? (n1 / 2 + 1 + 3) / 4 : (n1 + 7) / 8;
  int const ipc = m->rows == ROWS_V2 ? (real ? RowsV2Shape<true>::IPC : RowsV2Shape<false>::IPC) : 0;
  m->n_rows_ctas = ipc ? ((real ? n1 / 2 + 1 : n1) + ipc - 1) / ipc : m->rows == ROWS_2S ? (n1 + 7) / 8 : m->n_item_ctas;
}

static int master_setup(kgpu_master *m) {
  int const n1 = m->sp.n1, n2 = m->sp.n2;
  bool const real = m->in_type == KGPU_REAL;
  auto root = [](long e, long n) {
    long double const ang = -2.0L * M_PIl * (long double)(e % n) / (long double)n;
    return make_float2((float)cosl(ang), (float)sinl(ang));
  };
  if (real) {
    std::vector<float2> rootD((size_t)n2);
    for (int k2 = 0; k2 < n2; k2++) {
      long double const ang = -M_PIl * (long double)k2 / (long double)n2;
      rootD[(size_t)k2] = make_float2((float)cosl(ang), (float)sinl(ang));
    }
    if (upload(&m->d_rootD, rootD)) return -1;
  }
  if (real && m->rows == ROWS_V2) {
    std::vector<float2> tC((size_t)n1 / 2 + 1);
    for (int k1 = 0; k1 <= n1 / 2; k1++) tC[(size_t)k1] = root(k1, 2 * m->nc);
    if (upload(&m->d_rootC, tC)) return -1;
  }
  if (m->cols == COLS_R36) {
    static int const kPow[10] = {1, 2, 3, 4, 5, 6, 12, 18, 24, 30};
    std::vector<float2> t0(360), tA((size_t)n2 * 36), tB((size_t)(n2 + 8) * 10, make_float2(0.f, 0.f));
    for (int e = 0; e < 10; e++)
      for (int j = 0; j < 36; j++) t0[(size_t)e * 36 + j] = root((long)j * kPow[e], 1296);
    for (long c = 0; c < n2; c++) {
      for (int t = 0; t < 36; t++) tA[(size_t)c * 36 + t] = root(c * t, m->nc);
      for (int e = 0; e < 10; e++) tB[(size_t)c * 10 + e] = root(c * 36 * kPow[e], m->nc);
    }
    if (upload(&m->d_tw0, t0) || upload(&m->d_twA, tA) || upload(&m->d_twB, tB)) return -1;
    for (int f = 0; f < 3; f++)
      if (allow_smem((const void *)cols_r36_kernel(m, f), ColsR36Shape::smem) ||
          allow_smem((const void *)cols_r36_tma_kernel(m, f), ColsR36Shape::smem))
        return -1;
  }
  if (m->cols == COLS_2S) {
    constexpr int RA = 25, RB = 32, RC = 25, RD = 25;
    std::vector<float2> t0((size_t)Cols2s::TW0, make_float2(0.f, 0.f)), tA((size_t)n2 * RA),
        tB((size_t)(n2 + 8) * Cols2s::NP1, make_float2(0.f, 0.f)), r0((size_t)Rows2s::TW0, make_float2(0.f, 0.f));
    for (int e = 0; e < Cols2s::NP0; e++)
      for (int j = 0; j < RB; j++) t0[(size_t)e * RB + j] = root((long)j * Pow<RA>::exponent(e), n1);
    for (long c = 0; c < n2; c++) {
      for (int t = 0; t < RA; t++) tA[(size_t)c * RA + t] = root(c * t, m->nc);
      for (int e = 0; e < Cols2s::NP1; e++) tB[(size_t)c * Cols2s::NP1 + e] = root(c * RA * Pow<RB>::exponent(e), m->nc);
    }
    for (int e = 0; e < Rows2s::NP0; e++)
      for (int j = 0; j < RD; j++) r0[(size_t)e * RD + j] = root((long)j * Pow<RC>::exponent(e), n2);
    if (upload(&m->d_tw0, t0) || upload(&m->d_twA, tA) || upload(&m->d_twB, tB) || upload(&m->d_rtw0, r0)) return -1;
    for (int f = 0; f < 3; f++)
      if (allow_smem((const void *)cols_2s_kernel(f), Cols2s::smem)) return -1;
    if (allow_smem((const void *)fwd_rows_2s<25, 25>, Rows2s::smem)) return -1;
  }
  if (m->rows == ROWS_V2 && allow_smem((const void *)rows_v2_kernel(m), rows_v2_smem(m))) return -1;
  if (m->ext) {
    if (allow_smem((const void *)fwd_cols_ext<0>, m->smem1) || allow_smem((const void *)fwd_cols_ext<1>, m->smem1) ||
        allow_smem((const void *)fwd_rows_ext, m->smem2))
      return -1;
  } else if (allow_smem((const void *)fwd_cols_kernel<0>, m->smem1) || allow_smem((const void *)fwd_cols_kernel<1>, m->smem1) ||
             allow_smem((const void *)fwd_rows_kernel, m->smem2)) {
    return -1;
  }
  return 0;
}

extern "C" void kgpu_master_destroy(kgpu_master *m) {
  if (!m) return;
  if (m->ext) {
    free_tile_plan(m->xplan1);
    free_tile_plan(m->xplan2);
  }
  cudaFree(m->d_rootD);
  cudaFree(m->d_rootC);
  cudaFree(m->d_tw0);
  cudaFree(m->d_twA);
  cudaFree(m->d_twB);
  cudaFree(m->d_rtw0);
  cudaFree(m->mid.p);
  cudaFree(m->d_notch);
  kgpu_master_destroy(m->bs);
  cudaFree(m->blue.d_b);
  cudaFree(m->b_in.p);
  cudaFree(m->b_out.p);
  delete m;
}
extern "C" int kgpu_master_points(kgpu_master const *m) { return m ? m->N : -1; }
extern "C" int kgpu_master_bins(kgpu_master const *m) { return m ? m->bins : -1; }
extern "C" long kgpu_master_spec_stride(kgpu_master const *m) { return m ? m->spec_stride : -1; }

static std::string describe_text(kgpu_master const *m) {
  auto radices = [](std::vector<int> const &v) {
    std::string r;
    for (size_t i = 0; i < v.size(); i++) r += std::to_string(v[i]) + (i + 1 < v.size() ? "," : "");
    return r;
  };
  auto plan_of = [m](int len) { return m->ext ? choose_radices_ext(len) : choose_radices(len); };
  std::string const rc = m->cols == COLS_2S ? "25,32" : m->cols == COLS_R36 ? "36,36" : radices(plan_of(m->sp.n1));
  std::string const rr = m->rows == ROWS_2S ? "25,25" : m->rows == ROWS_V2 ? "10,25,5" : radices(plan_of(m->sp.n2));
  size_t const s1 = m->cols == COLS_2S ? Cols2s::smem : m->cols == COLS_R36 ? ColsR36Shape::smem : m->smem1;
  size_t const s2 = m->rows == ROWS_2S ? Rows2s::smem : m->rows == ROWS_V2 ? rows_v2_smem(m) : m->smem2;
  char const *kc = m->ext ? "fwd_cols_ext" : m->cols == COLS_2S ? "fwd_cols_2s" : m->cols == COLS_R36 ? "fwd_cols_r36" : "fwd_cols_kernel";
  char const *kr = m->ext ? "fwd_rows_ext" : m->rows == ROWS_2S ? "fwd_rows_2s" : m->rows == ROWS_V2 ? "fwd_rows_v2" : "fwd_rows_kernel";
  char buf[512];
  snprintf(buf, sizeof buf, "N=%d %s, %ld-point complex two-pass %d x %d; cols radices [%s] rows radices [%s]; smem %zu/%zu B; "
           "grids %d/%d CTAs per block; kernels %s + %s", m->N, m->in_type == KGPU_REAL ? "real" : "complex", m->nc, m->sp.n1,
           m->sp.n2, rc.c_str(), rr.c_str(), s1, s2, (m->sp.n2 + kTile - 1) / kTile, m->n_rows_ctas, kc, kr);
  return buf;
}
static std::string bluestein_text(Bluestein const &b, char const *in, char const *out) {
  kgpu_master inner;
  master_shape(&inner, (int)b.P, 1, KGPU_COMPLEX, b.sp, false);
  std::string const t = describe_text(&inner);
  return t.substr(t.find(", ") + 2) + " around " + in + ", bluestein_mul_kernel, " + out;
}
static std::string describe_bluestein(int N, int in_type, Bluestein const &b) {
  return "N=" + std::to_string(N) + (in_type == KGPU_REAL ? " real" : " complex") + ", bluestein P=" + std::to_string(b.P) +
         ": " + bluestein_text(b, "bluestein_in_kernel", "bluestein_out_kernel");
}

extern "C" int kgpu_master_describe(kgpu_master const *m, char *buf, int buflen) {
  if (!m || !buf) return -1;
  std::string const t = m->bs ? describe_bluestein(m->N, m->in_type, m->blue) : describe_text(m);
  snprintf(buf, (size_t)buflen, "%s", t.c_str());
  return 0;
}

static constexpr long kBluesteinScratchCap = 128L << 20;
enum MasterPath { MP_DIRECT = 0, MP_EXTENDED = 1, MP_BLUESTEIN = 2 };
struct MasterPlan {
  MasterPath path;
  long nc;
  Split2 sp;
  Bluestein blue;
};
#define KGPU_EXT_FACTORS "2, 3, 5, 7, 11, 13, 17, 19, 23"
static int master_plan(int L, int M, int in_type, MasterPath ceiling, char const *who, MasterPlan *pl) {
  if (L < 1 || M < 1 || (in_type != KGPU_REAL && in_type != KGPU_COMPLEX))
    return fail("%s: bad arguments L=%d M=%d type=%d", who, L, M, in_type);
  long const N = (long)L + M - 1;
  if (N > INT32_MAX) return fail("%s: N=L+M-1 is too large (L=%d M=%d)", who, L, M);
  if (in_type == KGPU_REAL && ((N & 1) || (L & 1)))
    return fail("%s: REAL input needs even L and even N=L+M-1 (got L=%d N=%ld)", who, L, N);
  long const nc = (in_type == KGPU_COMPLEX) ? N : N / 2;
  pl->nc = nc;
  if (smooth7(nc) && forward_split(nc, false, &pl->sp)) {
    pl->path = MP_DIRECT;
    return 0;
  }
  if (ceiling >= MP_EXTENDED && smooth23(nc) && forward_split(nc, true, &pl->sp)) {
    pl->path = MP_EXTENDED;
    return 0;
  }
  if (ceiling == MP_BLUESTEIN) {
    if (bluestein_shape(nc, &pl->blue)) {
      pl->path = MP_BLUESTEIN;
      return 0;
    }
    return fail("%s: %ld points need a Bluestein transform of at least %ld points, more than the forward pair splits (at "
                "most 3500 x 3500)", who, nc, 2 * nc - 1);
  }
  bool const ext = ceiling == MP_EXTENDED && !smooth7(nc);
  char const *const name = ext ? "kgpu_master_create_ex" : "kgpu_master_create";
  char const *const factors = ext ? KGPU_EXT_FACTORS : "2,3,5,7";
  if (ext) {
    long rest = nc;
    for (long p : {2, 3, 5, 7, 11, 13, 17, 19, 23})
      while (rest % p == 0) rest /= p;
    if (rest != 1) {
      long q = 29;
      while (q * q <= rest && rest % q) q++;
      if (rest % q) q = rest;
      return fail("%s: %ld points have the prime factor %ld (accepted factors %s)", name, nc, q, factors);
    }
  }
  Split2 sp;
  if (!(ext ? choose_split_ext(nc, &sp) : choose_split(nc, &sp)))
    return fail("%s: %ld points cannot be split into two plannable lengths (factors %s; <= %d)", name, nc, factors, kMaxTileLen);
  kgpu_master m;
  master_shape(&m, L, M, in_type, sp, ext);
  return fail("%s: %ld points split as %d x %d, which needs %zu / %zu B of shared memory (at most %d; factors %s)", name, nc,
              sp.n1, sp.n2, m.smem1, m.smem2, kChanSmemLimit, factors);
}

static kgpu_master *master_create(int L, int M, int in_type, MasterPath ceiling, char const *who) {
  MasterPlan pl;
  if (master_plan(L, M, in_type, ceiling, who, &pl)) return nullptr;
  kgpu_master *m = new kgpu_master;
  bool ok;
  if (pl.path == MP_BLUESTEIN) {
    master_geometry(m, L, M, in_type);
    m->blue = pl.blue;
    m->b_chunk = (int)std::max(1L, kBluesteinScratchCap / (long)(sizeof(float2) * (size_t)(pl.blue.P + 3)));
    m->bs = kgpu_master_create((int)pl.blue.P, 1, KGPU_COMPLEX);
    ok = m->bs && bluestein_upload(&m->blue) == 0;
  } else {
    master_shape(m, L, M, in_type, pl.sp, pl.path == MP_EXTENDED);
    if (m->ext) {
      m->plan1 = m->plan2 = -1;
      ok = make_tile_plan(pl.sp.n1, choose_radices_ext(pl.sp.n1), m->xplan1) == 0 &&
           make_tile_plan(pl.sp.n2, choose_radices_ext(pl.sp.n2), m->xplan2) == 0;
    } else {
      m->plan1 = get_tile_plan(pl.sp.n1);
      m->plan2 = get_tile_plan(pl.sp.n2);
      ok = m->plan1 >= 0 && m->plan2 >= 0;
    }
    ok = ok && master_setup(m) == 0;
  }
  if (!ok) {
    fail("%s: %s", who, std::string(g_err).c_str());
    kgpu_master_destroy(m);
    return nullptr;
  }
  return m;
}

extern "C" kgpu_master *kgpu_master_create(int L, int M, int in_type) {
  return master_create(L, M, in_type, MP_DIRECT, "kgpu_master_create");
}
extern "C" kgpu_master *kgpu_master_create_ex(int L, int M, int in_type) {
  return master_create(L, M, in_type, MP_EXTENDED, "kgpu_master_create_ex");
}
extern "C" kgpu_master *kgpu_master_create_any(int L, int M, int in_type) {
  return master_create(L, M, in_type, MP_BLUESTEIN, "kgpu_master_create_any");
}

extern "C" int kgpu_master_plan(int L, int M, int in_type, char *buf, int buflen) {
  MasterPlan pl;
  if (master_plan(L, M, in_type, MP_BLUESTEIN, "kgpu_master_plan", &pl)) return -1;
  if (buf && buflen > 0) {
    std::string t;
    if (pl.path == MP_BLUESTEIN) {
      t = describe_bluestein(L + M - 1, in_type, pl.blue);
    } else {
      kgpu_master m;
      master_shape(&m, L, M, in_type, pl.sp, pl.path == MP_EXTENDED);
      t = describe_text(&m);
    }
    snprintf(buf, (size_t)buflen, "%s", t.c_str());
  }
  return (int)pl.path;
}

static bool cols_tma_fits(kgpu_master const *m, void const *d_in, int fmt) {
  long const point = fmt == KGPU_FMT_I16 ? 4 : 8;
  long const hop = m->in_type == KGPU_REAL ? m->L / 2 : m->L;
  return m->cols == COLS_R36 && (uintptr_t)d_in % 16 == 0 && hop * point % 16 == 0 && 8L * m->sp.n2 % 16 == 0 &&
         m->sp.n1 % 2 == 0;
}

extern "C" int kgpu_cols_tma_fits(int L, int M, int in_type, int fmt, const void *d_in) {
  MasterPlan pl;
  if (master_plan(L, M, in_type, MP_BLUESTEIN, "kgpu_cols_tma_fits", &pl)) return -1;
  if (pl.path != MP_DIRECT) return 0;
  kgpu_master m;
  master_shape(&m, L, M, in_type, pl.sp, false);
  return cols_tma_fits(&m, d_in, fmt) ? 1 : 0;
}

static int cols_tma_map(kgpu_master const *m, void const *d_in, int fmt, int nblocks, CUtensorMap *map) {
  static PFN_cuTensorMapEncodeTiled const encode = [] {
    void *fn = nullptr;
    cudaDriverEntryPointQueryResult q;
    if (cudaGetDriverEntryPoint("cuTensorMapEncodeTiled", &fn, cudaEnableDefault, &q) != cudaSuccess ||
        q != cudaDriverEntryPointSuccess)
      fn = nullptr;
    return (PFN_cuTensorMapEncodeTiled)fn;
  }();
  if (!encode) return fail("kgpu_forward: the driver has no cuTensorMapEncodeTiled");
  bool const i16 = fmt == KGPU_FMT_I16;
  cuuint64_t const n1 = (cuuint64_t)m->sp.n1, n2 = (cuuint64_t)m->sp.n2;
  cuuint64_t const hop = (cuuint64_t)(m->in_type == KGPU_REAL ? m->L / 2 : m->L);
  cuuint64_t const dim[3] = {2 * n2, i16 ? n1 / 2 : n1, (cuuint64_t)nblocks};
  cuuint64_t const stride[2] = {8 * n2, hop * (i16 ? 4 : 8)};
  cuuint32_t const box[3] = {(cuuint32_t)(i16 ? ColsR36Tma::I16_BOX_WORDS : 16), ColsR36Tma::BOX_ROWS, 1};
  cuuint32_t const unit[3] = {1, 1, 1};
  CUresult const r = encode(map, i16 ? CU_TENSOR_MAP_DATA_TYPE_UINT32 : CU_TENSOR_MAP_DATA_TYPE_FLOAT32, 3, const_cast<void *>(d_in),
                            dim, stride, box, unit, CU_TENSOR_MAP_INTERLEAVE_NONE, CU_TENSOR_MAP_SWIZZLE_NONE,
                            CU_TENSOR_MAP_L2_PROMOTION_L2_128B, CU_TENSOR_MAP_FLOAT_OOB_FILL_NONE);
  if (r != CUDA_SUCCESS) return fail("kgpu_forward: cuTensorMapEncodeTiled failed (%d)", (int)r);
  return 0;
}

static int forward_span(kgpu_master *m, const void *d_in, int fmt, float scale, int derandomize, int nblocks, void *d_spec,
                        void *d_stats, cudaStream_t st, float2 *mid) {
  bool const use_static = g_static_on.load() != 0;
  ColsKernel const cols = use_static ? m->cols : COLS_GENERIC;
  RowsKernel const rows = use_static ? m->rows : ROWS_GENERIC;
  Pass1Args a1;
  a1.in = d_in;
  a1.hop = (m->in_type == KGPU_REAL) ? m->L / 2 : m->L;
  a1.n1 = m->sp.n1;
  a1.n2 = m->sp.n2;
  a1.nc = m->nc;
  a1.plan = m->plan1;
  a1.pitch = m->pitch1;
  a1.scale = scale;
  a1.derandomize = derandomize;
  a1.first_new = (m->in_type == KGPU_REAL) ? (m->M - 1) / 2 : (m->M - 1);
  a1.mid = mid;
  a1.stats = (fmt == KGPU_FMT_I16) ? (IngestStats *)d_stats : nullptr;
  a1.out_scale = (fmt == KGPU_FMT_I16 ? scale : 1.0f) * (m->halved ? 0.5f : 1.0f);
  a1.mid_ld = use_static ? m->mid_ld : m->sp.n2;
  int const f = (fmt != KGPU_FMT_I16) ? 0 : ((derandomize || a1.stats) ? 2 : 1);
  dim3 const g1((unsigned)((m->sp.n2 + kTile - 1) / kTile), (unsigned)nblocks);
  {
    ProfScope ps(K_FWD_COLS, st);
    switch (cols) {
      case COLS_2S:
        cols_2s_kernel(f)<<<g1, Cols2s::T, Cols2s::smem, st>>>(a1, Cols2sTables{m->d_tw0, m->d_twA, m->d_twB});
        break;
      case COLS_R36:
        if (cols_tma_on() && cols_tma_fits(m, d_in, fmt)) {
          CUtensorMap map;
          if (cols_tma_map(m, d_in, fmt, nblocks, &map)) return -1;
          cols_r36_tma_kernel(m, f)<<<g1, ColsR36Shape::T, ColsR36Shape::smem, st>>>(a1, ColsR36Tables{m->d_tw0, m->d_twA, m->d_twB}, map);
        } else {
          cols_r36_kernel(m, f)<<<g1, ColsR36Shape::T, ColsR36Shape::smem, st>>>(a1, ColsR36Tables{m->d_tw0, m->d_twA, m->d_twB});
        }
        break;
      case COLS_GENERIC:
        if (m->ext && f) fwd_cols_ext<1><<<g1, kFwdThreads, m->smem1, st>>>(a1, m->xplan1);
        else if (m->ext) fwd_cols_ext<0><<<g1, kFwdThreads, m->smem1, st>>>(a1, m->xplan1);
        else if (f) fwd_cols_kernel<1><<<g1, kFwdThreads, m->smem1, st>>>(a1);
        else fwd_cols_kernel<0><<<g1, kFwdThreads, m->smem1, st>>>(a1);
        break;
    }
  }
  g_launches++;
  Pass2Args a2;
  a2.mid = mid;
  a2.n1 = m->sp.n1;
  a2.n2 = m->sp.n2;
  a2.nc = m->nc;
  a2.plan = m->plan2;
  a2.pitch = m->pitch2;
  a2.real_split = (m->in_type == KGPU_REAL);
  a2.rootD = m->d_rootD;
  a2.spec = (float2 *)d_spec;
  a2.spec_stride = m->spec_stride;
  a2.mid_ld = a1.mid_ld;
  dim3 const g2((unsigned)(rows == ROWS_GENERIC ? m->n_item_ctas : m->n_rows_ctas), (unsigned)nblocks);
  {
    ProfScope ps(K_FWD_ROWS, st);
    switch (rows) {
      case ROWS_2S:
        fwd_rows_2s<25, 25><<<g2, Rows2s::T, Rows2s::smem, st>>>(a2, m->d_rtw0);
        break;
      case ROWS_V2:
        rows_v2_kernel(m)<<<g2, rows_v2_threads(m), rows_v2_smem(m), st>>>(a2, FwdTables{m->d_rootC});
        break;
      case ROWS_GENERIC:
        if (m->ext) fwd_rows_ext<<<g2, kFwdThreads, m->smem2, st>>>(a2, m->xplan2);
        else fwd_rows_kernel<<<g2, kFwdThreads, m->smem2, st>>>(a2);
        break;
    }
  }
  g_launches++;
  CUDA_OK(cudaGetLastError());
  return 0;
}

static int bluestein_conv(kgpu_master *im, Bluestein const &b, float2 *a, int rows, float2 *y, cudaStream_t st) {
  if (kgpu_forward(im, a, KGPU_FMT_F32, 1.0f, 0, rows, y, nullptr, st) != 0) return -1;
  {
    ProfScope ps(K_FWD_COLS, st);
    bluestein_mul_kernel<<<dim3((unsigned)((b.P + kBluesteinThreads - 1) / kBluesteinThreads), (unsigned)rows), kBluesteinThreads, 0,
                           st>>>(y, im->spec_stride, b.d_b, (int)b.P, a);
  }
  g_launches++;
  return kgpu_forward(im, a, KGPU_FMT_F32, 1.0f, 0, rows, y, nullptr, st);
}

static int bluestein_chain(kgpu_master *im, Bluestein const &b, BluesteinInArgs a, BluesteinOutArgs o, float2 *bin, float2 *bout,
                           cudaStream_t st) {
  a.nc = o.nc = b.n;
  a.P = b.P;
  a.out = bin;
  o.y = bout;
  o.y_stride = im->spec_stride;
  o.inv_p = 1.0 / (double)b.P;
  o.nblocks = a.nblocks;
  long const bins = o.real_split ? b.n + 1 : b.n;
  {
    ProfScope ps(K_FWD_COLS, st);
    bluestein_in_kernel<<<(unsigned)((b.P + kBluesteinThreads - 1) / kBluesteinThreads), kBluesteinThreads, 0, st>>>(a);
  }
  g_launches++;
  if (bluestein_conv(im, b, bin, a.nblocks, bout, st)) return -1;
  {
    ProfScope ps(K_FWD_ROWS, st);
    bluestein_out_kernel<<<(unsigned)((bins + kBluesteinThreads - 1) / kBluesteinThreads), kBluesteinThreads, 0, st>>>(o);
  }
  g_launches++;
  return 0;
}

static int bluestein_forward(kgpu_master *m, const void *d_in, int fmt, float scale, int derandomize, int nblocks, void *d_spec,
                             void *d_stats, cudaStream_t st) {
  int const chunk = std::min(nblocks, m->b_chunk);
  if (grow(m->b_in, sizeof(float2) * (size_t)m->blue.P * (size_t)chunk, st, "kgpu_forward") ||
      grow(m->b_out, sizeof(float2) * (size_t)m->bs->spec_stride * (size_t)chunk, st, "kgpu_forward"))
    return -1;
  bool const i16 = fmt == KGPU_FMT_I16;
  if (i16 && d_stats) CUDA_OK(cudaMemsetAsync(d_stats, 0, sizeof(IngestStats) * (size_t)nblocks, st));
  bool const real = m->in_type == KGPU_REAL;
  BluesteinInArgs a{};
  a.hop = real ? m->L / 2 : m->L;
  a.first_new = real ? (m->M - 1) / 2 : (m->M - 1);
  a.i16 = i16;
  a.derandomize = i16 && derandomize;
  a.scale = scale;
  BluesteinOutArgs o{};
  o.real_split = real;
  o.spec_stride = m->spec_stride;
  size_t const pair = i16 ? sizeof(short2) : sizeof(float2);
  for (int b0 = 0; b0 < nblocks; b0 += chunk) {
    a.in = (char const *)d_in + pair * (size_t)a.hop * (size_t)b0;
    a.nblocks = std::min(chunk, nblocks - b0);
    a.stats = (i16 && d_stats) ? (IngestStats *)d_stats + b0 : nullptr;
    o.spec = (float2 *)d_spec + (size_t)m->spec_stride * (size_t)b0;
    if (bluestein_chain(m->bs, m->blue, a, o, (float2 *)m->b_in.p, (float2 *)m->b_out.p, st)) return -1;
  }
  CUDA_OK(cudaGetLastError());
  return 0;
}

extern "C" int kgpu_forward(kgpu_master *m, const void *d_in, int fmt, float scale, int derandomize, int nblocks,
                            void *d_spec, void *d_stats, void *stream) {
  if (!m || !d_in || !d_spec || nblocks < 1) return fail("kgpu_forward: bad arguments");
  cudaStream_t st = (cudaStream_t)stream;
  if (m->bs) return bluestein_forward(m, d_in, fmt, scale, derandomize, nblocks, d_spec, d_stats, st);
  size_t const mid = sizeof(float2) * (size_t)m->sp.n1 * (size_t)((m->sp.n2 + 15) / 16 * 16);
  if (grow(m->mid, mid * (size_t)nblocks, st, "kgpu_forward")) return -1;
  if (fmt == KGPU_FMT_I16 && d_stats) CUDA_OK(cudaMemsetAsync(d_stats, 0, sizeof(IngestStats) * (size_t)nblocks, st));
  return forward_span(m, d_in, fmt, scale, derandomize, nblocks, d_spec, d_stats, st, (float2 *)m->mid.p);
}

extern "C" int kgpu_master_set_notches(kgpu_master *m, int const *bins, double const *alpha, int n) {
  if (!m || n < 0) return fail("kgpu_master_set_notches: bad arguments");
  cudaFree(m->d_notch);
  m->d_notch = nullptr;
  m->n_notch = 0;
  if (n == 0) return 0;
  std::vector<NotchDev> v((size_t)n);
  m->notch_sequential = 0;
  for (int i = 0; i < n; i++) {
    if (bins[i] < 0 || bins[i] >= m->bins) return fail("kgpu_master_set_notches: bin %d out of range", bins[i]);
    v[(size_t)i] = {bins[i], 0, 0.0, 0.0, alpha[i]};
    for (int j = 0; j < i; j++)
      if (bins[j] == bins[i]) m->notch_sequential = 1;
  }
  CUDA_OK(cudaMalloc(&m->d_notch, sizeof(NotchDev) * (size_t)n));
  CUDA_OK(cudaMemcpy(m->d_notch, v.data(), sizeof(NotchDev) * (size_t)n, cudaMemcpyHostToDevice));
  m->n_notch = n;
  return 0;
}
extern "C" int kgpu_apply_notches(kgpu_master *m, void *d_spec, int nblocks, void *stream) {
  if (!m || !d_spec) return fail("kgpu_apply_notches: bad arguments");
  if (m->n_notch == 0) return 0;
  {
    ProfScope ps(K_NOTCH, (cudaStream_t)stream);
    notch_kernel<<<1, 32 * ((m->n_notch + 31) / 32), 0, (cudaStream_t)stream>>>(
        m->d_notch, m->n_notch, m->notch_sequential, (float2 *)d_spec, m->spec_stride, nblocks);
  }
  g_launches++;
  CUDA_OK(cudaGetLastError());
  return 0;
}

namespace {
double bessel_i0(double z) {
  double const q = z * z / 4;
  double sum = 1 + q, term = q;
  for (int k = 2; k < 40; k++) {
    term *= q / ((double)k * (double)k);
    sum += term;
    if (term < 1e-12 * sum) break;
  }
  return sum;
}
void cis_revolutions(double x, double *re, double *im) {
  double y = fmod(x, 2.0);
  if (y < 0) y += 2.0;
  int const quad = (int)floor(2.0 * y) & 3;
  double z = y - 0.5 * quad;
  bool const fold = z > 0.25;
  if (fold) z = 0.5 - z;
  double s = sin(M_PI * z), c = cos(M_PI * z);
  if (fold) std::swap(s, c);
  switch (quad) {
    case 0: *re = c; *im = s; break;
    case 1: *re = -s; *im = c; break;
    case 2: *re = -c; *im = -s; break;
    default: *re = s; *im = -c; break;
  }
}
int design_taps(int points, int olen, int master_points, bool master_real, double low, double high, double beta,
                std::vector<float2> &taps) {
  if (isnan(low) || isnan(high) || isnan(beta)) return -1;
  if (low > high) std::swap(low, high);
  low = std::min(std::max(low, -0.5), 0.5);
  high = std::min(std::max(high, -0.5), 0.5);
  int const M = points - olen + 1;
  if (M < 2) return -1;
  double const half_bw = (high == low) ? 1e-4 : fabs(high - low) / 2;
  double const centre = (high + low) / 2;
  std::vector<float> win((size_t)M);
  double const norm0 = 1.0 / bessel_i0(beta), step = 2.0 / (M - 1);
  for (int n = 0; n < M / 2; n++) {
    double const p = step * n - 1;
    win[(size_t)n] = win[(size_t)(M - 1 - n)] = (float)(bessel_i0(beta * sqrt(1 - p * p)) * norm0);
  }
  if (M & 1) win[(size_t)((M - 1) / 2)] = 1.0f;
  double wsum = 0;
  for (float w : win) wsum += w;
  if (wsum == 0 || !std::isfinite(wsum)) return -1;
  float const wgain = (float)(M / wsum);
  for (float &w : win) w *= wgain;
  taps.assign((size_t)points, make_float2(0.f, 0.f));
  std::vector<double> rr((size_t)M), cr((size_t)M), ci((size_t)M);
  double tap_sum = 0;
  for (int i = 0; i < M; i++) {
    double const n = i - (double)(M - 1) / 2;
    double const arg = 2 * half_bw * n;
    double const snc = (arg == 0) ? 1.0 : sin(M_PI * arg) / (M_PI * arg);
    rr[(size_t)i] = win[(size_t)i] * 2 * half_bw * snc;
    tap_sum += rr[(size_t)i];
    cis_revolutions(2 * centre * n, &cr[(size_t)i], &ci[(size_t)i]);
  }
  double const gain = (master_real ? M_SQRT2 : 1.0) / (tap_sum * master_points);
  for (int i = 0; i < M; i++) {
    float const tr = (float)(cr[(size_t)i] * rr[(size_t)i]), ti = (float)(ci[(size_t)i] * rr[(size_t)i]);
    taps[(size_t)i] = make_float2((float)((double)tr * gain), (float)((double)ti * gain));
  }
  return 0;
}
}

enum ChanPath { CP_DIRECT = 0, CP_WIDE = 1, CP_HUGE = 2, CP_EXTENDED = 3, CP_BLUESTEIN = 4 };
static char const *const kDefineName[] = {"kgpu_bank_define", "kgpu_bank_define_wide", "kgpu_bank_define_huge",
                                          "kgpu_bank_define_ext", "kgpu_bank_define_any"};
struct ChanRoute {
  ChanPath path;
  bool narrow;
  Split2 sp;
  Bluestein blue;
};

static int chan_route(int points, ChanPath ceiling, char const *who, ChanRoute *r) {
  long const big = factor_above7(points);
  ChanPath const size = points <= kMaxChanPoints ? CP_DIRECT : points <= kMaxWideChanPoints ? CP_WIDE : CP_HUGE;
  bool const too_long = points > kMaxHugeChanPoints;
  *r = ChanRoute{};
  r->path = big == 1 ? size : (big <= 23 && size != CP_HUGE) ? CP_EXTENDED : CP_BLUESTEIN;
  r->narrow = size == CP_DIRECT;
  if (too_long && ceiling == CP_BLUESTEIN)
    return fail("%s: %d-point inverse transform exceeds the %d-point maximum", who, points, kMaxHugeChanPoints);
  if (r->path == CP_BLUESTEIN && ceiling == CP_EXTENDED) {
    if (big > 23)
      return fail("kgpu_bank_define_ext: %d-point inverse transform has the prime factor %ld (prime factors up to 23 are served)",
                  points, big);
    return fail("kgpu_bank_define_ext: %d-point inverse transform has the prime factor %ld, served up to %d points only",
                points, big, kMaxWideChanPoints);
  }
  if (r->path > ceiling || too_long) {
    static int const kMaxPoints[] = {kMaxChanPoints, kMaxWideChanPoints, kMaxHugeChanPoints};
    ChanPath const c = std::min(ceiling, CP_HUGE);
    if (size > c || too_long)
      return fail("%s: %d-point inverse transform exceeds the %d-point maximum", kDefineName[c], points, kMaxPoints[c]);
    if (size == CP_DIRECT)
      return fail("kgpu_bank_define: %d-point transform cannot be planned (factors 2, 3, 5, 7; at most %d points)", points,
                  kMaxChanPoints);
    return fail("%s: %d-point transform cannot be split into two plannable lengths (factors 2, 3, 5, 7; each at most %d)",
                kDefineName[size], points, kMaxTileLen);
  }
  bool ok = true;
  if (r->path == CP_BLUESTEIN) ok = bluestein_shape(points, &r->blue);
  else if (!r->narrow) ok = r->path == CP_EXTENDED ? choose_split_ext(points, &r->sp) : choose_split(points, &r->sp);
  if (!ok) return fail("%s: %d-point transform has no split", who, points);
  return 0;
}

struct ChanGeom {
  ChanRoute r;
  int points = 0;
  int plan = -1;
  WideGeom wide{};
  HugeGeom huge{};
  TilePlan ext{};
  WideGeomExt wide_ext{};
};
static std::recursive_mutex g_geom_mu;
static std::map<std::pair<int, int>, ChanGeom> g_geom;

static ChanGeom const *chan_geom(int points, ChanRoute const &r);
static int factor_plan(int len, TilePlan *out) {
  ChanRoute r;
  if (chan_route(len, CP_EXTENDED, "factor_plan", &r)) return -1;
  ChanGeom const *g = chan_geom(len, r);
  if (!g) return -1;
  if (r.path == CP_EXTENDED) {
    *out = g->ext;
    return 0;
  }
  std::lock_guard<std::mutex> lk(g_plan_mu);
  *out = g_plans[(size_t)g->plan].host;
  return 0;
}

static ChanGeom const *chan_geom(int points, ChanRoute const &r) {
  int dev = 0;
  if (cudaGetDevice(&dev) != cudaSuccess) {
    fail("cudaGetDevice: %s", cudaGetErrorString(cudaGetLastError()));
    return nullptr;
  }
  std::lock_guard<std::recursive_mutex> lk(g_geom_mu);
  auto it = g_geom.find({dev, points});
  if (it != g_geom.end()) return &it->second;
  ChanGeom g;
  g.r = r;
  g.points = points;
  int const n1 = r.sp.n1, n2 = r.sp.n2;
  bool ok = true;
  switch (r.path) {
    case CP_DIRECT:
      g.plan = get_tile_plan(points);
      ok = g.plan >= 0;
      break;
    case CP_WIDE:
      g.wide = WideGeom{n1, n2, wide_pitch(n2), get_tile_plan(n1), get_tile_plan(n2), nullptr};
      ok = g.wide.plan1 >= 0 && g.wide.plan2 >= 0 && !wide_twiddles(g.wide, *host_tile_plan(g.wide.plan2));
      g.plan = g.wide.plan1;
      break;
    case CP_HUGE:
      g.huge = HugeGeom{n1, n2, huge_pitch(n1), huge_pitch(n2), get_tile_plan(n1), get_tile_plan(n2)};
      ok = g.huge.plan1 >= 0 && g.huge.plan2 >= 0;
      g.plan = g.huge.plan1;
      break;
    case CP_EXTENDED:
      g.plan = kPlanExt;
      if (r.narrow) {
        ok = make_tile_plan(points, choose_radices_ext(points), g.ext) == 0;
      } else {
// ... 1073 lines not shown
```

ka9q_radio_b200/csrc/static_kernels_v2.cuh:

```cuda
#pragma once
#include "static_kernels.cuh"

namespace kfft {

__device__ __forceinline__ void unpack_i16(int raw, int &lo, int &hi) {
  asm("prmt.b32 %0, %1, 0, 0x9910;" : "=r"(lo) : "r"(raw));
  hi = raw >> 16;
}
__device__ __forceinline__ float i32_to_f32(int v) {
  float f;
  asm("cvt.rn.f32.s32 %0, %1;" : "=f"(f) : "r"(v));
  return f;
}

template <bool REAL_SPLIT>
struct RowsV2Shape {
  using P = SPlan<1250, 10, 25, 5>;
  static constexpr int N2 = 1250, PITCH = 1250, GT = 256, SKEW = 2;
  static constexpr int NG = REAL_SPLIT ? 2 : 1, T = GT * NG, COLS = 8 * NG;
  static constexpr int IPC = REAL_SPLIT ? COLS / 2 : COLS;
  static constexpr int TW = (static_tw_count<P>() + 1) & ~1;
  static constexpr int TILE = COLS * PITCH + (NG - 1) * SKEW;
  static constexpr size_t smem = sizeof(float2) * (size_t)(TILE + TW);
  static __host__ __device__ constexpr int col_off(int c) { return c * PITCH + (c >> 3) * SKEW; }
};

__device__ constexpr float kRowsTw0[3][4][2] = {
    {{9.870916009e-01f, -1.601568460e-01f}, {9.486995935e-01f, -3.161789477e-01f}, {8.000617623e-01f, -5.999176502e-01f}, {2.801976204e-01f, -9.599423409e-01f}},
    {{9.486995935e-01f, -3.161789477e-01f}, {8.000617623e-01f, -5.999176502e-01f}, {2.801976204e-01f, -9.599423409e-01f}, {-8.429785967e-01f, -5.379471183e-01f}},
    {{8.858151436e-01f, -4.640382826e-01f}, {5.693368912e-01f, -8.221042752e-01f}, {-3.517109454e-01f, -9.361086488e-01f}, {-7.525988221e-01f, 6.584793329e-01f}},
};

template <bool REAL_SPLIT, int N1C = 0, bool HALVED = false>
__global__ void __launch_bounds__(RowsV2Shape<REAL_SPLIT>::T, REAL_SPLIT ? 1 : 2) fwd_rows_v2(Pass2Args const a, FwdTables const tb) {
  using S = RowsV2Shape<REAL_SPLIT>;
  using P = typename S::P;
  constexpr int N2 = S::N2, T = S::T, GT = S::GT, COLS = S::COLS, IPC = S::IPC;
  constexpr int R0 = 10, S0 = 125, R1 = 25, NSUB1 = 125, S1 = 5, R2 = 5;
  extern __shared__ __align__(16) unsigned char smem_raw[];
  float2 *tile = reinterpret_cast<float2 *>(smem_raw);
  float2 *s_tw = tile + S::TILE;
  __shared__ __align__(8) uint64_t bars[COLS];
  __shared__ __align__(8) uint64_t tbar;
  TilePlan const &pl = c_plans[a.plan];
  int const tid = threadIdx.x, lane = tid & 31, warp = tid >> 5;
  int const blk = gridDim.y - 1 - blockIdx.y;
  int const n1 = N1C ? N1C : a.n1;
  int const item0 = blockIdx.x * IPC;
  auto row_of = [&](int col) -> int {
    RowItem const it = row_item(item0 + (REAL_SPLIT ? col >> 1 : col), n1, REAL_SPLIT);
    if (REAL_SPLIT) {
      if ((col & 1) == 0) return it.kind != kRowEmpty ? it.row_a : -1;
      return it.kind == kRowPair ? it.row_b : -1;
    }
    return it.kind == kRowPlain ? it.row_a : -1;
  };
  if (lane == 0) {
    int const row = row_of(warp);
    mbar_init(&bars[warp], 1);
    if (warp == 0) mbar_init(&tbar, 1);
    mbar_fence_init();
    if (row >= 0) {
      mbar_expect_tx(&bars[warp], N2 * 8);
      bulk_g2s(tile + S::col_off(warp), a.mid + ((long)blk * n1 + row) * a.mid_ld, N2 * 8, &bars[warp]);
    }
    if (warp == 0) {
      constexpr uint32_t TWB = (uint32_t)S::TW * 8u;
      mbar_expect_tx(&tbar, TWB);
      bulk_g2s(s_tw, pl.tw, TWB, &tbar);
    }
  }
  __syncthreads();
  int const g = tid / GT;
  int const c = (tid & 7) + 8 * g, ul = (tid % GT) >> 3;
  auto group_sync = [&] {
    if (S::NG == 1) __syncthreads();
    else asm volatile("bar.sync %0, %1;" ::"r"(1 + g), "n"(GT) : "memory");
  };
  bool const col_ok = row_of(c) >= 0;
  mbar_wait(&tbar, 0);
  if (col_ok) mbar_wait(&bars[c], 0);
  float2 *mycol = tile + S::col_off(c);

  if (col_ok) {
    float2 base[4];
#pragma unroll
    for (int q = 0; q < 4; q++) base[q] = s_tw[((1 << q) - 1) * S0 + ul];
#pragma unroll
    for (int it = 0; it < 4; it++) {
      int const j = ul + (GT / 8) * it;
      if (it < 3 || j < S0) {
        float2 *p = mycol + j;
        float2 x[R0], w[R0];
#pragma unroll
        for (int m = 0; m < R0; m++) x[m] = p[m * S0];
#pragma unroll
        for (int q = 0; q < 4; q++)
          w[1 << q] = it == 0 ? base[q] : cmul(base[q], make_float2(kRowsTw0[it > 0 ? it - 1 : 0][q][0], kRowsTw0[it > 0 ? it - 1 : 0][q][1]));
        w[3] = cmul(w[2], w[1]);
        w[5] = cmul(w[4], w[1]);
        w[6] = cmul(w[4], w[2]);
        w[7] = cmul(w[4], w[3]);
        w[9] = cmul(w[8], w[1]);
        Dft<R0, false>::run(x);
        p[0] = x[0];
#pragma unroll
        for (int t = 1; t < R0; t++) p[t * S0] = cmul(x[t], w[t]);
      }
    }
  }
  group_sync();
  if (col_ok) {
    float2 const *tw1 = s_tw + P::tw_off(1);
#pragma unroll 1
    for (int u = ul; u < N2 / R1; u += GT / 8) {
      int const b = u / S1, j = u - b * S1;
      float2 *p = mycol + b * NSUB1 + j;
      float2 x[R1];
#pragma unroll
      for (int m = 0; m < R1; m++) x[m] = p[m * S1];
      Dft<R1, false>::run(x);
#pragma unroll
      for (int t = 1; t < R1; t++) x[t] = cmul(x[t], tw1[(t - 1) * S1 + j]);
#pragma unroll
      for (int t = 0; t < R1; t++) p[t * S1] = x[t];
    }
  }
  constexpr int UQ = T / IPC;
  int const i = tid % IPC, uq = tid / IPC;
  RowItem const it = row_item(item0 + i, n1, REAL_SPLIT);
  float2 rootC = make_float2(1.f, 0.f), rd[4];
  bool self_item = false;
  if (REAL_SPLIT) {
    self_item = it.kind == kRowSelf0 || it.kind == kRowSelfMid;
    if (it.kind == kRowPair) rootC = __ldg(tb.rootC + it.row_a);
#pragma unroll
    for (int q = 0; q < 4; q++) {
      int const u = uq + UQ * q;
      int const t0 = u / 25, t1 = u - t0 * 25;
      rd[q] = (it.kind == kRowPair && u < N2 / R2) ? __ldg(a.rootD + t0 + 10 * t1) : make_float2(1.f, 0.f);
    }
  }
  int const has_self = __syncthreads_or(self_item);

  float2 *spec = a.spec + (long)blk * a.spec_stride;
  float const hf = HALVED ? 1.0f : 0.5f;
  if (!REAL_SPLIT) {
    if (col_ok) {
      float2 *dst = spec + row_of(c);
#pragma unroll 1
      for (int u = ul; u < N2 / R2; u += GT / 8) {
        int const t0 = u / 25, t1 = u - t0 * 25;
        int const kb = t0 + 10 * t1;
        float2 const *p = mycol + u * R2;
        float2 x[R2];
#pragma unroll
        for (int m = 0; m < R2; m++) x[m] = p[m];
        Dft<R2, false>::run(x);
        float2 *d = dst + (long)n1 * kb;
#pragma unroll
        for (int t = 0; t < R2; t++) d[(long)n1 * 250 * t] = x[t];
      }
    }
    return;
  }
  int const nc = N1C ? N1C * N2 : (int)a.nc;
  if (it.kind == kRowPair) {
    float2 const *ca = tile + S::col_off(2 * i), *cb = tile + S::col_off(2 * i + 1);
#pragma unroll
    for (int q = 0; q < 4; q++) {
      int const u = uq + UQ * q;
      if (u >= N2 / R2) break;
      int const t0 = u / 25, t1 = u - t0 * 25;
      int const kb = t0 + 10 * t1;
      float2 const wkb = cmul(rootC, rd[q]);
      float2 za[R2], zb[R2];
      float2 const *pa = ca + u * R2, *pb = cb + (N2 / R2 - 1 - u) * R2;
      float2 *pk = spec + (it.row_a + n1 * kb), *pm = spec + (nc - it.row_a - n1 * kb);
#pragma unroll
      for (int m = 0; m < R2; m++) {
        za[m] = pa[m];
        zb[m] = pb[m];
      }
      Dft<R2, false>::run(za);
      Dft<R2, false>::run(zb);
#pragma unroll
      for (int t = 0; t < R2; t++) {
        float2 const A = za[t], B = zb[R2 - 1 - t];
        float2 const w = (t == 0) ? wkb : cmul(wkb, wroot<10>(t));
        float2 const E = HALVED ? make_float2(A.x + B.x, A.y - B.y) : make_float2(0.5f * (A.x + B.x), 0.5f * (A.y - B.y));
        float2 const O = HALVED ? make_float2(A.x - B.x, A.y + B.y) : make_float2(0.5f * (A.x - B.x), 0.5f * (A.y + B.y));
        float2 const Pp = cmul(w, O);
        pk[(long)n1 * 250 * t] = make_float2(E.x + Pp.y, E.y - Pp.x);
        pm[-(long)n1 * 250 * t] = make_float2(E.x - Pp.y, -(E.y + Pp.x));
      }
    }
  }
  if (!has_self) return;
  for (int s = 0; s < IPC; s++) {
    RowItem const its = row_item(item0 + s, n1, true);
    if (its.kind != kRowSelf0 && its.kind != kRowSelfMid) continue;
    float2 *col = tile + S::col_off(2 * s);
    for (int u = tid; u < N2 / R2; u += T) {
      float2 x[R2];
#pragma unroll
      for (int m = 0; m < R2; m++) x[m] = col[u * R2 + m];
      Dft<R2, false>::run(x);
#pragma unroll
      for (int m = 0; m < R2; m++) col[u * R2 + m] = x[m];
    }
  }
  __syncthreads();
  for (int s = 0; s < IPC; s++) {
    RowItem const its = row_item(item0 + s, n1, true);
    if (its.kind != kRowSelf0 && its.kind != kRowSelfMid) continue;
    float2 const *col = tile + S::col_off(2 * s);
    float2 const rC = __ldg(tb.rootC + its.row_a);
    bool const self0 = its.kind == kRowSelf0;
    int const kend = self0 ? N2 / 2 + 1 : (N2 + 1) / 2;
    for (int k2 = tid; k2 < kend; k2 += T) {
      int const k2m = self0 ? (k2 == 0 ? 0 : N2 - k2) : N2 - 1 - k2;
      float2 const A = col[static_slot<P>(k2)], B = col[static_slot<P>(k2m)];
      float2 const w = cmul(rC, __ldg(a.rootD + k2));
      float2 const E = make_float2(hf * (A.x + B.x), hf * (A.y - B.y));
      float2 const O = make_float2(hf * (A.x - B.x), hf * (A.y + B.y));
      float2 const Pp = cmul(w, O);
      int const k = its.row_a + n1 * k2;
      spec[k] = make_float2(E.x + Pp.y, E.y - Pp.x);
      if (nc - k != k) spec[nc - k] = make_float2(E.x - Pp.y, -(E.y + Pp.x));
    }
  }
}

template <class P, bool OSC = false>
__global__ void __launch_bounds__(kChanWarps * 32) chan_v2(ChanArgs const a) {
  static_assert(P::nst == 2, "two-stage plans only");
  extern __shared__ __align__(16) unsigned char smem_raw[];
  __shared__ __align__(8) uint64_t bars[kChanWarps];
  __shared__ __align__(8) uint64_t tbar;
  constexpr int NS = P::len, TOP = (NS + 1) / 2, R0 = P::rad(0), R1 = P::rad(1), S0 = NS / R0;
  static_assert(S0 == R1 && NS % 2 == 0, "plan shape");
  constexpr int XS = NS + 4;
  int const lane = threadIdx.x & 31, warp = threadIdx.x >> 5;
  int const oi = blockIdx.x * kChanWarps + warp;
  float2 *s_tw = reinterpret_cast<float2 *>(smem_raw) + kChanWarps * (NS + XS);
  bool const active = oi < a.norder;
  ChanDesc d;
  d.plan = -1;
  if (active) d = a.desc[a.order ? a.order[oi] : a.chan_base + oi];
  if (threadIdx.x == 0) {
    int p0 = -1;
    for (int w = 0; w < kChanWarps && p0 < 0; w++) {
      int const o = blockIdx.x * kChanWarps + w;
      if (o < a.norder) p0 = a.desc[a.order ? a.order[o] : a.chan_base + o].plan;
    }
    mbar_init(&tbar, 1);
    mbar_fence_init();
    if (p0 >= 0) {
      constexpr uint32_t TWB = (uint32_t)((static_tw_count<P>() + 1) & ~1) * 8u;
      mbar_expect_tx(&tbar, TWB);
      bulk_g2s(s_tw, c_plans[p0].tw, TWB, &tbar);
    }
  }
  __syncthreads();
  if (!active || d.plan < 0) return;
  int const blk = blockIdx.y;
  float2 *col = reinterpret_cast<float2 *>(smem_raw) + warp * (NS + XS);
  float2 *xs = col + NS;
  float2 const *X = a.spec + (long)blk * a.spec_stride;
  float2 const *R = a.resp + d.resp_off;
  float2 *dst = a.out + (long)blk * a.out_stride + d.out_off;
  if (d.ncopy <= 0) {
    for (int i = lane; i < d.olen; i += 32) dst[i] = make_float2(0.f, 0.f);
    if ((d.flags & kChanOsc) && a.power && lane == 0) a.power[(long)blk * a.power_stride + (a.order ? a.order[oi] : a.chan_base + oi)] = 0.f;
    mbar_wait(&tbar, 0);
    return;
  }
  int const qlo = d.dir > 0 ? d.q0 : d.q0 - (d.ncopy - 1);
  bool const wraps = a.wrap && (d.q0 + d.ncopy > a.m_bins);
  int const qa = qlo & ~1;
  if (!wraps) {
    int const qhi = qlo + d.ncopy - 1;
    uint32_t const nx = (uint32_t)(((qhi - qa + 1) + 1) & ~1);
    if (lane == 0) {
      mbar_init(&bars[warp], 1);
      mbar_fence_init();
      mbar_expect_tx(&bars[warp], nx * 8 + NS * 8);
      bulk_g2s(xs, X + qa, nx * 8, &bars[warp]);
      bulk_g2s(col, R, NS * 8, &bars[warp]);
    }
    __syncwarp();
    mbar_wait(&bars[warp], 0);
  } else {
    for (int i = lane; i < NS; i += 32) col[i] = __ldg(R + i);
    for (int u = lane; u < d.ncopy; u += 32) {
      int q = d.q0 + u;
      if (q >= a.m_bins) q -= a.m_bins;
      xs[u] = __ldg(X + q);
    }
    __syncwarp();
  }
  mbar_wait(&tbar, 0);
  auto product = [&](int wp) -> float2 {
    int t = wp - TOP;
    if (t < 0) t += NS;
    int const u = t - d.zlead;
    bool const live = (u >= 0 && u < d.ncopy && wp != TOP);
    int const xi = wraps ? u : (d.q0 + d.dir * u - qa);
    float2 x = xs[live ? xi : 0];
    if (d.dir < 0) x.y = -x.y;
    float2 const v = cmul(x, col[wp]);
    return live ? v : make_float2(0.f, 0.f);
  };
  if (d.flags & kChanIsb) {
    for (int wp = lane; wp < NS; wp += 32) col[wp] = product(wp);
    __syncwarp();
    for (int p = 1 + lane; p < NS / 2; p += 32) {
      float2 const pos = col[p], neg = col[NS - p];
      col[p] = make_float2(pos.x + neg.x, pos.y - neg.y);
      col[NS - p] = make_float2(neg.x - pos.x, neg.y + pos.y);
    }
    if (lane == 0) {
      col[0] = make_float2(0.f, 0.f);
      col[TOP] = make_float2(0.f, 0.f);
    }
    __syncwarp();
    static_stage<P, true, 0, true, 1>(col, s_tw, lane);
    __syncwarp();
  } else if (lane < S0) {
    float2 x[R0];
#pragma unroll
    for (int m = 0; m < R0; m++) x[m] = product(lane + S0 * m);
    Dft<R0, true>::run(x);
    col[lane] = x[0];
#pragma unroll
    for (int t = 1; t < R0; t++) col[lane + S0 * t] = cmulc(x[t], s_tw[(t - 1) * S0 + lane]);
  }
  __syncwarp();
  bool const osc = OSC && (d.flags & kChanOsc) != 0;
  float pw = 0.f;
  int const ci = a.order ? a.order[oi] : a.chan_base + oi;
  if (lane < R0) {
    float2 x[R1];
#pragma unroll
    for (int m = 0; m < R1; m++) x[m] = col[R1 * lane + m];
    Dft<R1, true>::run(x);
    int const first = NS - d.olen;
    if (!OSC || !osc) {
#pragma unroll
      for (int t = 0; t < R1; t++) {
        int const n = lane + R0 * t;
        if (n >= first) dst[n - first] = x[t];
      }
    } else if (OSC) {
      ChanAux const ax = a.aux[ci];
      long const k = a.block0 + blk - ax.osc_epoch;
#pragma unroll
      for (int t = 0; t < R1; t++) {
        int const n = lane + R0 * t;
        if (n >= first) {
          float2 const v = osc_rotate(x[t], osc_phase_cycles(ax, k, d.olen, n - first));
          dst[n - first] = v;
          pw += v.x * v.x + v.y * v.y;
        }
      }
    }
  }
  if (OSC && osc && a.power) {
    pw = warp_sum(pw);
    if (lane == 0) a.power[(long)blk * a.power_stride + ci] = pw / (float)d.olen;
  }
}

}
```

Baseline: 99330.

## Fuse forward column and row FFT passes into one ticketed persistent-style kernel

Adds a fused forward kernel that hands out work items through an atomic ticket counter. Column-pass tiles for block b+1 are interleaved with row-pass items for block b, and row items spin on per-block release/acquire counters until that block's columns are finished. This removes the separate launch and the full-grid barrier between the two passes, and lets the intermediate stay hot in L2. An optional mode discards the intermediate L2 lines after they are consumed. The costs are spin-wait stalls, a memset of the counters on every call, a 1-CTA-per-SM launch bound, and idle threads in row items.

```diff
diff --git a/include/ka9q_gpu.h b/include/ka9q_gpu.h
--- a/include/ka9q_gpu.h
+++ b/include/ka9q_gpu.h
@@ -146,6 +146,12 @@
 int kgpu_use_static_kernels(int on);
 int kgpu_use_cols_tma(int on);
 int kgpu_cols_tma_fits(int L, int M, int in_type, int fmt, const void *d_in);
+int kgpu_use_fused_forward(int on);
+int kgpu_fused_forward_fits(int L, int M, int in_type, int fmt, const void *d_in);
+int kgpu_fused_forward_options(int lead, int discard);
+int kgpu_fused_shape(int *out);
+int kgpu_fused_schedule(int nblocks, int lead, int ticket, int *out);
+long kgpu_fused_discards(int blk, int idx, long *lines, long max);
 
 int kgpu_plan_radices(int len, int *radices, int max);
 int kgpu_plan_split(long n, int *n1, int *n2);
diff --git a/ka9q_radio_b200/capi.py b/ka9q_radio_b200/capi.py
--- a/ka9q_radio_b200/capi.py
+++ b/ka9q_radio_b200/capi.py
@@ -101,6 +101,13 @@
     L.kgpu_use_static_kernels.argtypes = [i]
     L.kgpu_use_cols_tma.argtypes = [i]
     L.kgpu_cols_tma_fits.argtypes = [i, i, i, i, vp]
+    L.kgpu_use_fused_forward.argtypes = [i]
+    L.kgpu_fused_forward_fits.argtypes = [i, i, i, i, vp]
+    L.kgpu_fused_forward_options.argtypes = [i, i]
+    L.kgpu_fused_shape.argtypes = [vp]
+    L.kgpu_fused_schedule.argtypes = [i, i, i, vp]
+    L.kgpu_fused_discards.argtypes = [i, i, vp, l]
+    L.kgpu_fused_discards.restype = l
     L.kgpu_profile_enable.argtypes = [i]
     L.kgpu_profile_name.argtypes = [i]
     L.kgpu_profile_name.restype = C.c_char_p
diff --git a/ka9q_radio_b200/csrc/fft_static.cuh b/ka9q_radio_b200/csrc/fft_static.cuh
--- a/ka9q_radio_b200/csrc/fft_static.cuh
+++ b/ka9q_radio_b200/csrc/fft_static.cuh
@@ -142,6 +142,8 @@
                ::"r"(smem_u32(dst)), "l"(map), "r"(x), "r"(y), "r"(z), "r"(smem_u32(bar))
                : "memory");
 }
+__device__ __forceinline__ void fence_proxy_async_global() { asm volatile("fence.proxy.async.global;" ::: "memory"); }
+__device__ __forceinline__ void discard_l2_line(void *p) { asm volatile("discard.global.L2 [%0], 128;" ::"l"(p) : "memory"); }
 __device__ __forceinline__ void mbar_wait(uint64_t *bar, uint32_t parity) {
   asm volatile(
       "{\n\t.reg .pred p;\n\t"
diff --git a/ka9q_radio_b200/csrc/fwd_cols_r36.cuh b/ka9q_radio_b200/csrc/fwd_cols_r36.cuh
--- a/ka9q_radio_b200/csrc/fwd_cols_r36.cuh
+++ b/ka9q_radio_b200/csrc/fwd_cols_r36.cuh
@@ -65,17 +65,15 @@
   for (int t = 1; t < R; t++) d[t * BLK] = cmul(x[t], r36_power(wb, wa, t));
 }
 
-template <int FMT, int N2C, bool TMA>
-__device__ __forceinline__ void fwd_cols_r36_body(Pass1Args const &a, ColsR36Tables const &tb, CUtensorMap const *tmap) {
+template <int FMT, int N2C, bool TMA, class Sync>
+__device__ __forceinline__ void fwd_cols_r36_body(Pass1Args const &a, ColsR36Tables const &tb, CUtensorMap const *tmap,
+                                                  unsigned char *smem_raw, uint64_t &tbar, int tid, int c0, int blk,
+                                                  Sync const &sync) {
   constexpr int R = 36, BLK = ColsR36Shape::BLK, CP = ColsR36Shape::CP;
-  extern __shared__ __align__(16) unsigned char smem_raw[];
   float2 *tile = reinterpret_cast<float2 *>(smem_raw);
   float2 *s_tw0 = tile + 8 * CP;
   float2 *s_twB = s_tw0 + 360;
-  __shared__ __align__(8) uint64_t tbar;
-  int const tid = threadIdx.x;
   int const c = tid & 7, ul = tid >> 3;
-  int const c0 = blockIdx.x * 8, blk = blockIdx.y;
   int const n2 = N2C ? N2C : a.n2;
   int const ld = N2C ? (N2C + 15) / 16 * 16 : a.mid_ld;
   int const ncols = min(8, n2 - c0);
@@ -105,7 +103,7 @@
     bulk_g2s(s_tw0, tb.tw0, 360 * 8, &tbar);
     bulk_g2s(s_twB, tb.twB + (long)c0 * 10, 80 * 8, &tbar);
   }
-  __syncthreads();
+  sync();
   float2 const twA = col_ok ? ldg_stream_f2(tb.twA + (long)n2g * 36 + ul) : make_float2(1.f, 0.f);
 
   unsigned long long energy = 0;
@@ -129,7 +127,7 @@
       }
       Dft<R, false>::run(x);
     }
-    __syncthreads();
+    sync();
     if (col_ok) r36_stage0_store(x, s_tw0, mycol + ul, ul);
   } else if (col_ok) {
     float2 x[R];
@@ -162,7 +160,7 @@
       atomicAdd(&a.stats[blk].clips, clips);
     }
   }
-  __syncthreads();
+  sync();
 
   if (col_ok) {
     float2 x[R];
@@ -190,12 +188,18 @@
 
 template <int FMT, int N2C>
 __global__ void __launch_bounds__(ColsR36Shape::T, 2) fwd_cols_r36(Pass1Args const a, ColsR36Tables const tb) {
-  fwd_cols_r36_body<FMT, N2C, false>(a, tb, nullptr);
+  extern __shared__ __align__(16) unsigned char smem_raw[];
+  __shared__ __align__(8) uint64_t tbar;
+  fwd_cols_r36_body<FMT, N2C, false>(a, tb, nullptr, smem_raw, tbar, threadIdx.x, blockIdx.x * 8, blockIdx.y,
+                                     [] { __syncthreads(); });
 }
 template <int FMT, int N2C>
 __global__ void __launch_bounds__(ColsR36Shape::T, 2)
     fwd_cols_r36_tma(Pass1Args const a, ColsR36Tables const tb, const __grid_constant__ CUtensorMap tmap) {
-  fwd_cols_r36_body<FMT, N2C, true>(a, tb, &tmap);
-}
-
-}
+  extern __shared__ __align__(16) unsigned char smem_raw[];
+  __shared__ __align__(8) uint64_t tbar;
+  fwd_cols_r36_body<FMT, N2C, true>(a, tb, &tmap, smem_raw, tbar, threadIdx.x, blockIdx.x * 8, blockIdx.y,
+                                    [] { __syncthreads(); });
+}
+
+}
diff --git a/ka9q_radio_b200/csrc/fwd_fused.cuh b/ka9q_radio_b200/csrc/fwd_fused.cuh
--- /dev/null
+++ b/ka9q_radio_b200/csrc/fwd_fused.cuh
@@ -0,0 +1,96 @@
+#pragma once
+#include "fwd_cols_r36.cuh"
+#include "static_kernels_v2.cuh"
+
+namespace kfft {
+
+struct FusedShape {
+  static constexpr int N1 = 1296, N2 = 1250;
+  static constexpr int TILES = (N2 + 7) / 8;
+  static constexpr int NC = (TILES + 1) / 2;
+  static constexpr int NR = (N1 / 2 + 1 + RowsV2Shape<true>::IPC - 1) / RowsV2Shape<true>::IPC;
+  static constexpr int T = 2 * ColsR36Shape::T;
+  static constexpr int RT = RowsV2Shape<true>::T;
+  static constexpr size_t smem = 2 * ColsR36Shape::smem > RowsV2Shape<true>::smem ? 2 * ColsR36Shape::smem : RowsV2Shape<true>::smem;
+  static constexpr int DEFAULT_LEAD = 40;
+  static_assert(ColsR36Shape::smem % 16 == 0, "the second tile's memory 16-byte aligned");
+  static_assert(T % 32 == 0 && ColsR36Shape::T % 32 == 0 && RT % 32 == 0, "whole warps per tile and per R item");
+};
+
+enum FusedKind : int { kFusedCol = 0, kFusedRow = 1 };
+struct FusedItem {
+  int kind, blk, idx;
+};
+
+__host__ __device__ __forceinline__ FusedItem fused_item(int t, int nblocks, int lead) {
+  using F = FusedShape;
+  if (t < F::NC) return {kFusedCol, 0, t};
+  t -= F::NC;
+  int const b = t / (F::NR + F::NC), p = t - b * (F::NR + F::NC);
+  if (b >= nblocks - 1) return {kFusedRow, nblocks - 1, t - (nblocks - 1) * (F::NR + F::NC)};
+  if (p < lead) return {kFusedCol, b + 1, p};
+  int const q = p - lead, m = F::NC - lead;
+  if (q < 2 * m) return (q & 1) ? FusedItem{kFusedCol, b + 1, lead + q / 2} : FusedItem{kFusedRow, b, q / 2};
+  return {kFusedRow, b, q - m};
+}
+
+struct FusedArgs {
+  unsigned *ctr;
+  int nblocks, lead;
+  int discard;
+};
+
+__device__ __forceinline__ void red_release_gpu_add(unsigned *p, unsigned v) {
+  asm volatile("red.release.gpu.global.add.u32 [%0], %1;" ::"l"(p), "r"(v) : "memory");
+}
+__device__ __forceinline__ unsigned ld_acquire_gpu(unsigned const *p) {
+  unsigned v;
+  asm volatile("ld.acquire.gpu.global.u32 %0, [%1];" : "=r"(v) : "l"(p) : "memory");
+  return v;
+}
+
+template <int FMT>
+__global__ void __launch_bounds__(FusedShape::T, 1)
+    fwd_fused_r36_v2(Pass1Args const a1, ColsR36Tables const t1, Pass2Args const a2, FwdTables const t2, FusedArgs const f,
+                     const __grid_constant__ CUtensorMap tmap) {
+  using F = FusedShape;
+  extern __shared__ __align__(16) unsigned char smem_raw[];
+  __shared__ __align__(8) uint64_t bars[RowsV2Shape<true>::COLS];
+  __shared__ __align__(8) uint64_t tbar[2];
+  __shared__ int s_ticket;
+  int const tid = threadIdx.x;
+  if (tid == 0) s_ticket = (int)atomicAdd(f.ctr, 1u);
+  __syncthreads();
+  FusedItem const it = fused_item(s_ticket, f.nblocks, f.lead);
+  if (it.kind == kFusedCol) {
+    int const h = tid >= ColsR36Shape::T, tile = 2 * it.idx + h;
+    if (tile < F::TILES)
+      fwd_cols_r36_body<FMT, F::N2, true>(a1, t1, &tmap, smem_raw + h * ColsR36Shape::smem, tbar[h], tid - h * ColsR36Shape::T,
+                                           tile * 8, it.blk, [h] {
+                                             asm volatile("bar.sync %0, %1;" ::"r"(1 + h), "n"(ColsR36Shape::T) : "memory");
+                                           });
+    __syncthreads();
+    if (tid == 0) {
+      __threadfence();
+      red_release_gpu_add(f.ctr + 1 + fused_item(s_ticket, f.nblocks, f.lead).blk, 1u);
+    }
+    return;
+  }
+  if (tid >= F::RT) return;
+  auto sync = [] { asm volatile("bar.sync 3, %0;" ::"n"(F::RT) : "memory"); };
+  auto sync_or = [](int p) {
+    int r;
+    asm volatile("{\n\t.reg .pred q, o;\n\tsetp.ne.s32 q, %1, 0;\n\tbar.red.or.pred o, 3, %2, q;\n\tselp.s32 %0, 1, 0, o;\n\t}"
+                 : "=r"(r)
+                 : "r"(p), "n"(F::RT)
+                 : "memory");
+    return r;
+  };
+  if (tid == 0)
+    while (ld_acquire_gpu(f.ctr + 1 + it.blk) < (unsigned)F::NC) __nanosleep(64);
+  sync();
+  fwd_rows_v2_body<true, F::N1, true, true>(a2, t2, smem_raw, bars, tbar[0], tid, it.blk, it.idx * RowsV2Shape<true>::IPC,
+                                            sync, sync_or, f.discard);
+}
+
+}
diff --git a/ka9q_radio_b200/csrc/fwd_kernels.cuh b/ka9q_radio_b200/csrc/fwd_kernels.cuh
--- a/ka9q_radio_b200/csrc/fwd_kernels.cuh
+++ b/ka9q_radio_b200/csrc/fwd_kernels.cuh
@@ -156,7 +156,7 @@
   int row_b;
 };
 
-__device__ __forceinline__ RowItem row_item(int p, int n1, bool real_split) {
+__host__ __device__ __forceinline__ RowItem row_item(int p, int n1, bool real_split) {
   RowItem it;
   if (!real_split) {
     it.kind = p < n1 ? kRowPlain : kRowEmpty;
diff --git a/ka9q_radio_b200/csrc/kgpu.cu b/ka9q_radio_b200/csrc/kgpu.cu
--- a/ka9q_radio_b200/csrc/kgpu.cu
+++ b/ka9q_radio_b200/csrc/kgpu.cu
@@ -23,6 +23,7 @@
 #include "static_kernels.cuh"
 #include "static_kernels_v2.cuh"
 #include "fwd_cols_r36.cuh"
+#include "fwd_fused.cuh"
 #include "fwd_2s.cuh"
 #include "spectrum_kernels.cuh"
 #include "bluestein_master.cuh"
@@ -51,6 +52,21 @@
     char const *e = getenv("KA9Q_COLS_TMA");
     g_cols_tma.compare_exchange_strong(v, (e && *e) ? (atoi(e) != 0) : 1);
     v = g_cols_tma.load();
+  }
+  return v != 0;
+}
+static std::atomic<int> g_fused{-1};
+static std::atomic<int> g_fused_lead{FusedShape::DEFAULT_LEAD}, g_fused_discard{0};
+extern "C" int kgpu_use_fused_forward(int on) {
+  g_fused.store(on != 0);
+  return 0;
+}
+static bool fused_on() {
+  int v = g_fused.load();
+  if (v < 0) {
+    char const *e = getenv("KA9Q_FUSED_FWD");
+    g_fused.compare_exchange_strong(v, (e && *e) ? (atoi(e) != 0) : 1);
+    v = g_fused.load();
   }
   return v != 0;
 }
@@ -112,8 +128,8 @@
   return 0;
 }
 
-enum KernelId { K_FWD_COLS = 0, K_FWD_ROWS, K_CHAN, K_NOTCH, K_RESPONSE, K_NOISE, K_COUNT };
-static char const *const kKernelNames[K_COUNT] = {"fwd_cols", "fwd_rows", "chan", "notch", "response_fft", "noise"};
+enum KernelId { K_FWD_COLS = 0, K_FWD_ROWS, K_CHAN, K_NOTCH, K_RESPONSE, K_NOISE, K_FWD_FUSED, K_COUNT };
+static char const *const kKernelNames[K_COUNT] = {"fwd_cols", "fwd_rows", "chan", "notch", "response_fft", "noise", "fwd_fused"};
 struct ProfRec {
   cudaEvent_t a, b;
   int kid;
@@ -750,6 +766,7 @@
   float2 *d_tw0 = nullptr, *d_twA = nullptr, *d_twB = nullptr;
   float2 *d_rtw0 = nullptr;
   StreamBuf mid;
+  StreamBuf fused_ctr;
   size_t smem1 = 0, smem2 = 0;
   bool ext = false;
   TilePlan xplan1{}, xplan2{};
@@ -785,6 +802,15 @@
 static RowsV2Fn rows_v2_kernel(kgpu_master const *m) {
   if (m->in_type == KGPU_REAL) return m->halved ? fwd_rows_v2<true, 1296, true> : fwd_rows_v2<true, 0, false>;
   return m->n1c ? fwd_rows_v2<false, 1296, false> : fwd_rows_v2<false, 0, false>;
+}
+static bool fused_pair(kgpu_master const *m) {
+  return m->in_type == KGPU_REAL && m->cols == COLS_R36 && m->rows == ROWS_V2 && m->halved && m->n2c == FusedShape::N2 &&
+         m->n1c == FusedShape::N1 && m->mid_ld % 16 == 0;
+}
+using FusedFn = void (*)(Pass1Args, ColsR36Tables, Pass2Args, FwdTables, FusedArgs, CUtensorMap);
+static FusedFn fused_kernel(int f) {
+  static FusedFn const k[3] = {fwd_fused_r36_v2<0>, fwd_fused_r36_v2<1>, fwd_fused_r36_v2<2>};
+  return k[f];
 }
 static int rows_v2_threads(kgpu_master const *m) { return m->in_type == KGPU_REAL ? RowsV2Shape<true>::T : RowsV2Shape<false>::T; }
 static size_t rows_v2_smem(kgpu_master const *m) {
@@ -898,6 +924,9 @@
     if (allow_smem((const void *)fwd_rows_2s<25, 25>, Rows2s::smem)) return -1;
   }
   if (m->rows == ROWS_V2 && allow_smem((const void *)rows_v2_kernel(m), rows_v2_smem(m))) return -1;
+  if (fused_pair(m))
+    for (int f = 0; f < 3; f++)
+      if (allow_smem((const void *)fused_kernel(f), FusedShape::smem)) return -1;
   if (m->ext) {
     if (allow_smem((const void *)fwd_cols_ext<0>, m->smem1) || allow_smem((const void *)fwd_cols_ext<1>, m->smem1) ||
         allow_smem((const void *)fwd_rows_ext, m->smem2))
@@ -922,6 +951,7 @@
   cudaFree(m->d_twB);
   cudaFree(m->d_rtw0);
   cudaFree(m->mid.p);
+  cudaFree(m->fused_ctr.p);
   cudaFree(m->d_notch);
   kgpu_master_destroy(m->bs);
   cudaFree(m->blue.d_b);
@@ -1102,6 +1132,62 @@
   return cols_tma_fits(&m, d_in, fmt) ? 1 : 0;
 }
 
+static bool fused_fits(kgpu_master const *m, void const *d_in, int fmt) { return fused_pair(m) && cols_tma_fits(m, d_in, fmt); }
+
+extern "C" int kgpu_fused_forward_fits(int L, int M, int in_type, int fmt, const void *d_in) {
+  MasterPlan pl;
+  if (master_plan(L, M, in_type, MP_BLUESTEIN, "kgpu_fused_forward_fits", &pl)) return -1;
+  if (pl.path != MP_DIRECT) return 0;
+  kgpu_master m;
+  master_shape(&m, L, M, in_type, pl.sp, false);
+  return fused_fits(&m, d_in, fmt) ? 1 : 0;
+}
+
+extern "C" int kgpu_fused_forward_options(int lead, int discard) {
+  if (lead < 0 || lead > FusedShape::NC) return fail("kgpu_fused_forward_options: lead %d outside 0..%d", lead, FusedShape::NC);
+  g_fused_lead.store(lead);
+  g_fused_discard.store(discard != 0);
+  return 0;
+}
+
+extern "C" int kgpu_fused_shape(int *out) {
+  if (!out) return fail("kgpu_fused_shape: bad arguments");
+  out[0] = FusedShape::NC;
+  out[1] = FusedShape::NR;
+  out[2] = FusedShape::N1;
+  out[3] = (FusedShape::N2 + 15) / 16 * 16;
+  out[4] = FusedShape::DEFAULT_LEAD;
+  return 0;
+}
+
+extern "C" int kgpu_fused_schedule(int nblocks, int lead, int ticket, int *out) {
+  if (nblocks < 1 || lead < 0 || lead > FusedShape::NC || ticket < 0 || ticket >= nblocks * (FusedShape::NC + FusedShape::NR) ||
+      !out)
+    return fail("kgpu_fused_schedule: bad arguments");
+  FusedItem const it = fused_item(ticket, nblocks, lead);
+  out[0] = it.kind;
+  out[1] = it.blk;
+  out[2] = it.idx;
+  out[3] = it.kind == kFusedRow ? it.blk : -1;
+  out[4] = it.kind == kFusedRow ? FusedShape::NC : 0;
+  return 0;
+}
+
+extern "C" long kgpu_fused_discards(int blk, int idx, long *lines, long max) {
+  using S = RowsV2Shape<true>;
+  if (blk < 0 || idx < 0 || idx >= FusedShape::NR || max < 0) return fail("kgpu_fused_discards: bad arguments");
+  int const ld = (FusedShape::N2 + 15) / 16 * 16;
+  long n = 0;
+  for (int col = 0; col < S::COLS; col++) {
+    RowItem const it = row_item(idx * S::IPC + (col >> 1), FusedShape::N1, true);
+    int const row = (col & 1) == 0 ? (it.kind != kRowEmpty ? it.row_a : -1) : (it.kind == kRowPair ? it.row_b : -1);
+    if (row < 0) continue;
+    for (int l = 0; l < mid_row_lines(ld); l++, n++)
+      if (lines && n < max) lines[n] = mid_line(blk, FusedShape::N1, row, ld, l);
+  }
+  return n;
+}
+
 static int cols_tma_map(kgpu_master const *m, void const *d_in, int fmt, int nblocks, CUtensorMap *map) {
   static PFN_cuTensorMapEncodeTiled const encode = [] {
     void *fn = nullptr;
@@ -1126,6 +1212,45 @@
   return 0;
 }
 
+static Pass2Args rows_args(kgpu_master const *m, Pass1Args const &a1, void *d_spec) {
+  Pass2Args a2;
+  a2.mid = a1.mid;
+  a2.n1 = m->sp.n1;
+  a2.n2 = m->sp.n2;
+  a2.nc = m->nc;
+  a2.plan = m->plan2;
+  a2.pitch = m->pitch2;
+  a2.real_split = (m->in_type == KGPU_REAL);
+  a2.rootD = m->d_rootD;
+  a2.spec = (float2 *)d_spec;
+  a2.spec_stride = m->spec_stride;
+  a2.mid_ld = a1.mid_ld;
+  return a2;
+}
+
+static int fused_span(kgpu_master *m, const void *d_in, int fmt, int f, int nblocks, void *d_spec, cudaStream_t st,
+                      Pass1Args const &a1) {
+  using F = FusedShape;
+  size_t const ctr_bytes = sizeof(unsigned) * (size_t)(1 + nblocks);
+  if (grow(m->fused_ctr, ctr_bytes, st, "kgpu_forward")) return -1;
+  CUtensorMap map;
+  if (cols_tma_map(m, d_in, fmt, nblocks, &map)) return -1;
+  FusedArgs fa;
+  fa.ctr = (unsigned *)m->fused_ctr.p;
+  fa.nblocks = nblocks;
+  fa.lead = g_fused_lead.load();
+  fa.discard = g_fused_discard.load();
+  CUDA_OK(cudaMemsetAsync(fa.ctr, 0, ctr_bytes, st));
+  {
+    ProfScope ps(K_FWD_FUSED, st);
+    fused_kernel(f)<<<(unsigned)(nblocks * (F::NC + F::NR)), F::T, F::smem, st>>>(a1, ColsR36Tables{m->d_tw0, m->d_twA, m->d_twB},
+                                                                       rows_args(m, a1, d_spec), FwdTables{m->d_rootC}, fa, map);
+  }
+  g_launches++;
+  CUDA_OK(cudaGetLastError());
+  return 0;
+}
+
 static int forward_span(kgpu_master *m, const void *d_in, int fmt, float scale, int derandomize, int nblocks, void *d_spec,
                         void *d_stats, cudaStream_t st, float2 *mid) {
   bool const use_static = g_static_on.load() != 0;
@@ -1147,6 +1272,7 @@
   a1.out_scale = (fmt == KGPU_FMT_I16 ? scale : 1.0f) * (m->halved ? 0.5f : 1.0f);
   a1.mid_ld = use_static ? m->mid_ld : m->sp.n2;
   int const f = (fmt != KGPU_FMT_I16) ? 0 : ((derandomize || a1.stats) ? 2 : 1);
+  if (nblocks >= 2 && use_static && cols_tma_on() && fused_on() && fused_fits(m, d_in, fmt)) return fused_span(m, d_in, fmt, f, nblocks, d_spec, st, a1);
   dim3 const g1((unsigned)((m->sp.n2 + kTile - 1) / kTile), (unsigned)nblocks);
   {
     ProfScope ps(K_FWD_COLS, st);
@@ -1172,18 +1298,7 @@
     }
   }
   g_launches++;
-  Pass2Args a2;
-  a2.mid = mid;
-  a2.n1 = m->sp.n1;
-  a2.n2 = m->sp.n2;
-  a2.nc = m->nc;
-  a2.plan = m->plan2;
-  a2.pitch = m->pitch2;
-  a2.real_split = (m->in_type == KGPU_REAL);
-  a2.rootD = m->d_rootD;
-  a2.spec = (float2 *)d_spec;
-  a2.spec_stride = m->spec_stride;
-  a2.mid_ld = a1.mid_ld;
+  Pass2Args const a2 = rows_args(m, a1, d_spec);
   dim3 const g2((unsigned)(rows == ROWS_GENERIC ? m->n_item_ctas : m->n_rows_ctas), (unsigned)nblocks);
   {
     ProfScope ps(K_FWD_ROWS, st);
diff --git a/ka9q_radio_b200/csrc/static_kernels_v2.cuh b/ka9q_radio_b200/csrc/static_kernels_v2.cuh
--- a/ka9q_radio_b200/csrc/static_kernels_v2.cuh
+++ b/ka9q_radio_b200/csrc/static_kernels_v2.cuh
@@ -31,22 +31,24 @@
     {{8.858151436e-01f, -4.640382826e-01f}, {5.693368912e-01f, -8.221042752e-01f}, {-3.517109454e-01f, -9.361086488e-01f}, {-7.525988221e-01f, 6.584793329e-01f}},
 };
 
-template <bool REAL_SPLIT, int N1C = 0, bool HALVED = false>
-__global__ void __launch_bounds__(RowsV2Shape<REAL_SPLIT>::T, REAL_SPLIT ? 1 : 2) fwd_rows_v2(Pass2Args const a, FwdTables const tb) {
+__host__ __device__ constexpr int mid_row_lines(int mid_ld) { return mid_ld * 8 / 128; }
+__host__ __device__ constexpr long mid_line(int blk, int n1, int row, int mid_ld, int l) {
+  return ((long)blk * n1 + row) * mid_row_lines(mid_ld) + l;
+}
+
+template <bool REAL_SPLIT, int N1C, bool HALVED, bool FUSED, class Sync, class SyncOr>
+__device__ __forceinline__ void fwd_rows_v2_body(Pass2Args const &a, FwdTables const &tb, unsigned char *smem_raw,
+                                                 uint64_t *bars, uint64_t &tbar, int tid, int blk, int item0,
+                                                 Sync const &sync, SyncOr const &sync_or, bool discard = false) {
   using S = RowsV2Shape<REAL_SPLIT>;
   using P = typename S::P;
   constexpr int N2 = S::N2, T = S::T, GT = S::GT, COLS = S::COLS, IPC = S::IPC;
   constexpr int R0 = 10, S0 = 125, R1 = 25, NSUB1 = 125, S1 = 5, R2 = 5;
-  extern __shared__ __align__(16) unsigned char smem_raw[];
   float2 *tile = reinterpret_cast<float2 *>(smem_raw);
   float2 *s_tw = tile + S::TILE;
-  __shared__ __align__(8) uint64_t bars[COLS];
-  __shared__ __align__(8) uint64_t tbar;
   TilePlan const &pl = c_plans[a.plan];
-  int const tid = threadIdx.x, lane = tid & 31, warp = tid >> 5;
-  int const blk = gridDim.y - 1 - blockIdx.y;
+  int const lane = tid & 31, warp = tid >> 5;
   int const n1 = N1C ? N1C : a.n1;
-  int const item0 = blockIdx.x * IPC;
   auto row_of = [&](int col) -> int {
     RowItem const it = row_item(item0 + (REAL_SPLIT ? col >> 1 : col), n1, REAL_SPLIT);
     if (REAL_SPLIT) {
@@ -61,6 +63,7 @@
     if (warp == 0) mbar_init(&tbar, 1);
     mbar_fence_init();
     if (row >= 0) {
+      if (FUSED) fence_proxy_async_global();
       mbar_expect_tx(&bars[warp], N2 * 8);
       bulk_g2s(tile + S::col_off(warp), a.mid + ((long)blk * n1 + row) * a.mid_ld, N2 * 8, &bars[warp]);
     }
@@ -70,16 +73,20 @@
       bulk_g2s(s_tw, pl.tw, TWB, &tbar);
     }
   }
-  __syncthreads();
+  sync();
   int const g = tid / GT;
   int const c = (tid & 7) + 8 * g, ul = (tid % GT) >> 3;
   auto group_sync = [&] {
-    if (S::NG == 1) __syncthreads();
+    if (S::NG == 1) sync();
     else asm volatile("bar.sync %0, %1;" ::"r"(1 + g), "n"(GT) : "memory");
   };
   bool const col_ok = row_of(c) >= 0;
   mbar_wait(&tbar, 0);
   if (col_ok) mbar_wait(&bars[c], 0);
+  if (FUSED && discard && col_ok) {
+    char *const mid = const_cast<char *>(reinterpret_cast<char const *>(a.mid));
+    for (int l = ul; l < mid_row_lines(a.mid_ld); l += GT / 8) discard_l2_line(mid + 128 * mid_line(blk, n1, row_of(c), a.mid_ld, l));
+  }
   float2 *mycol = tile + S::col_off(c);
 
   if (col_ok) {
@@ -141,7 +148,7 @@
       rd[q] = (it.kind == kRowPair && u < N2 / R2) ? __ldg(a.rootD + t0 + 10 * t1) : make_float2(1.f, 0.f);
     }
   }
-  int const has_self = __syncthreads_or(self_item);
+  int const has_self = sync_or(self_item);
 
   float2 *spec = a.spec + (long)blk * a.spec_stride;
   float const hf = HALVED ? 1.0f : 0.5f;
@@ -210,7 +217,7 @@
       for (int m = 0; m < R2; m++) col[u * R2 + m] = x[m];
     }
   }
-  __syncthreads();
+  sync();
   for (int s = 0; s < IPC; s++) {
     RowItem const its = row_item(item0 + s, n1, true);
     if (its.kind != kRowSelf0 && its.kind != kRowSelfMid) continue;
@@ -230,6 +237,16 @@
       if (nc - k != k) spec[nc - k] = make_float2(E.x - Pp.y, -(E.y + Pp.x));
     }
   }
+}
+
+template <bool REAL_SPLIT, int N1C = 0, bool HALVED = false>
+__global__ void __launch_bounds__(RowsV2Shape<REAL_SPLIT>::T, REAL_SPLIT ? 1 : 2) fwd_rows_v2(Pass2Args const a, FwdTables const tb) {
+  extern __shared__ __align__(16) unsigned char smem_raw[];
+  __shared__ __align__(8) uint64_t bars[RowsV2Shape<REAL_SPLIT>::COLS];
+  __shared__ __align__(8) uint64_t tbar;
+  fwd_rows_v2_body<REAL_SPLIT, N1C, HALVED, false>(a, tb, smem_raw, bars, tbar, threadIdx.x, gridDim.y - 1 - blockIdx.y,
+                                                   blockIdx.x * RowsV2Shape<REAL_SPLIT>::IPC, [] { __syncthreads(); },
+                                                   [](int p) { return __syncthreads_or(p); });
 }
 
 template <class P, bool OSC = false>
```

After: 104,300, median of 6. 1.05x the previous value.
